# MrOlm/inStrain

Hardware: AMD Instinct MI355X
Metric: Gbp profiled/s (higher is better)
Workload: dtype u32

## Files before the change

### instrain_amd/csrc/isx_api.hip

```cpp
#include <algorithm>
#include <atomic>
#include <cmath>
#include <chrono>
#include <cstdlib>
#include <cstring>
#include <map>
#include <mutex>
#include <string>
#include <unordered_map>
#include <thread>
#include <type_traits>
#include <vector>
#include <unistd.h>
#include <sys/prctl.h>
#include <time.h>

#include "isx_batch.h"
#include "seg_encode.h"

static thread_local std::string g_err;
void isx_set_error(const std::string &msg) { g_err = msg; }

namespace {
struct BlockCache {
// ... 169 lines not shown
    std::lock_guard<std::mutex> lk(g_hreg_mu);
    for (size_t i = 0; i < g_hreg.size(); i++)
        if (g_hreg[i].a == a) {
            g_hreg.erase(g_hreg.begin() + (long)i);
            HIP_TRY(hipHostUnregister(const_cast<void *>(ptr)));
            return ISX_OK;
        }
    isx_set_error("isx_host_unregister: not a registered range");
    return ISX_ERR_ARG;
}

namespace {
__global__ void __launch_bounds__(256) k_copy_out(uint4 *__restrict__ dst, const uint4 *__restrict__ src, size_t n16)
{
    typedef uint32_t u32x4 __attribute__((ext_vector_type(4)));
    const size_t stride = (size_t)gridDim.x * blockDim.x;
    for (size_t i = (size_t)blockIdx.x * blockDim.x + threadIdx.x; i < n16; i += stride) {
        const u32x4 v = __builtin_nontemporal_load(reinterpret_cast<const u32x4 *>(src) + i);
        reinterpret_cast<u32x4 *>(dst)[i] = v;
    }
}
}

namespace {
template <class T>
__global__ void __launch_bounds__(256) k_copy_small(T *__restrict__ dst, const T *__restrict__ src, size_t n)
{
    const size_t stride = (size_t)gridDim.x * blockDim.x;
    for (size_t i = (size_t)blockIdx.x * blockDim.x + threadIdx.x; i < n; i += stride) dst[i] = src[i];
}
}

hipError_t isx_copy_to_host(void *hdst, const void *dsrc, size_t bytes, hipStream_t stream)
{
    static const size_t dma_min = [] { const char *e = getenv("ISX_D2H_DMA_MIN"); return e ? (size_t)atoll(e) : (size_t)1 << 20; }();
    return isx_copy_to_host_route(hdst, dsrc, bytes, stream, bytes < dma_min);
}

hipError_t isx_copy_to_host_route(void *hdst, const void *dsrc, size_t bytes, hipStream_t stream, bool by_kernel)
{
    if (!bytes) return hipSuccess;
    if (!by_kernel) return hipMemcpyAsync(hdst, dsrc, bytes, hipMemcpyDeviceToHost, stream);
    const uintptr_t both = reinterpret_cast<uintptr_t>(hdst) | reinterpret_cast<uintptr_t>(dsrc);
    size_t done = 0;
    if ((both & 15) == 0 && bytes >= 4096) {
        const size_t n16 = bytes / 16;
        const int blocks = (int)std::min<size_t>(128, (n16 + 1023) / 1024);
        hipLaunchKernelGGL(k_copy_out, dim3(blocks), dim3(256), 0, stream, static_cast<uint4 *>(hdst), static_cast<const uint4 *>(dsrc), n16);
        done = n16 * 16;
    }
    if (done < bytes) {
        const size_t rest = bytes - done;
        uint8_t *d = static_cast<uint8_t *>(hdst) + done;
        const uint8_t *s = static_cast<const uint8_t *>(dsrc) + done;
        const bool words = (((both | rest) & 3) == 0);
        const size_t n = words ? rest / 4 : rest;
        const int blocks = (int)std::min<size_t>(64, (n + 255) / 256);
        if (words) hipLaunchKernelGGL(k_copy_small<uint32_t>, dim3(blocks), dim3(256), 0, stream, reinterpret_cast<uint32_t *>(d), reinterpret_cast<const uint32_t *>(s), n);
        else hipLaunchKernelGGL(k_copy_small<uint8_t>, dim3(blocks), dim3(256), 0, stream, d, s, n);
    }
    return hipGetLastError();
}

namespace {
__global__ void __launch_bounds__(256) k_copy_counted(uint4 *__restrict__ dst, const uint4 *__restrict__ src, const uint32_t *cursor,
                                                      uint32_t base, uint32_t row_bytes, uint64_t cap_rows)
{
    const uint64_t rows = min((uint64_t)(*cursor - base), cap_rows);
    const uint64_t n16 = (rows * row_bytes + 15) / 16;
    const uint64_t stride = (uint64_t)gridDim.x * blockDim.x;
    for (uint64_t i = (uint64_t)blockIdx.x * blockDim.x + threadIdx.x; i < n16; i += stride) dst[i] = src[i];
}
}

hipError_t isx_copy_rows_to_host(void *hdst, const void *dsrc, const uint32_t *d_cursor, uint32_t base, uint32_t row_bytes,
                                 size_t cap_rows, hipStream_t stream)
{
    if (!cap_rows) return hipSuccess;
    if (((reinterpret_cast<uintptr_t>(hdst) | reinterpret_cast<uintptr_t>(dsrc)) & 15) != 0) return hipErrorInvalidValue;
    const size_t n16 = (cap_rows * row_bytes + 15) / 16;
    const int blocks = (int)std::min<size_t>(64, (n16 + 1023) / 1024);
    hipLaunchKernelGGL(k_copy_counted, dim3(std::max(blocks, 1)), dim3(256), 0, stream, static_cast<uint4 *>(hdst), static_cast<const uint4 *>(dsrc),
                       d_cursor, base, row_bytes, (uint64_t)cap_rows);
    return hipGetLastError();
}

namespace {
struct CopyJobs { uint4 *dst[ISX_COPY_JOBS]; const uint4 *src[ISX_COPY_JOBS]; uint32_t n16[ISX_COPY_JOBS]; uint32_t first[ISX_COPY_JOBS + 1]; int n; };
__global__ void __launch_bounds__(256) k_copy_multi(const CopyJobs J)
{
    int j = 0;
    while (j + 1 < J.n && blockIdx.x >= J.first[j + 1]) j++;
    const uint32_t nb = J.first[j + 1] - J.first[j], lb = blockIdx.x - J.first[j];
    for (uint32_t i = lb * 256u + threadIdx.x; i < J.n16[j]; i += nb * 256u) J.dst[j][i] = J.src[j][i];
}
}

hipError_t isx_copy_multi_to_host(const isx_copy_job *jobs, int n, hipStream_t stream)
{
    CopyJobs J{};
    uint32_t blocks = 0;
    for (int i = 0; i < n && J.n < ISX_COPY_JOBS; i++) {
        if (!jobs[i].bytes) continue;
        if (((reinterpret_cast<uintptr_t>(jobs[i].dst) | reinterpret_cast<uintptr_t>(jobs[i].src)) & 15) != 0 || jobs[i].bytes > ((size_t)1 << 35)) return hipErrorInvalidValue;
        const uint32_t n16 = (uint32_t)((jobs[i].bytes + 15) / 16);
        J.dst[J.n] = static_cast<uint4 *>(jobs[i].dst); J.src[J.n] = static_cast<const uint4 *>(jobs[i].src); J.n16[J.n] = n16;
        J.first[J.n] = blocks;
        blocks += std::max<uint32_t>(1, std::min<uint32_t>(64, (n16 + 1023) / 1024));
        J.n++;
    }
    if (!J.n) return hipSuccess;
    J.first[J.n] = blocks;
    hipLaunchKernelGGL(k_copy_multi, dim3(blocks), dim3(256), 0, stream, J);
    return hipGetLastError();
}

namespace {
struct ReadBack {
    uint8_t *pin = nullptr;
    size_t used = 0;
    struct Item { void *dst; size_t off, bytes; };
    std::vector<Item> items;
    bool batching = false;
    std::vector<isx_copy_job> jobs;
    static constexpr size_t CAP = (size_t)1 << 20;
    ~ReadBack() { if (pin) isx_pin_free(pin); }
};
thread_local ReadBack g_rb;
}

void isx_read_batch(bool on) { g_rb.batching = on; }

hipError_t isx_read_back(void *host_dst, const void *dsrc, size_t bytes, hipStream_t stream)
{
    if (!bytes) return hipSuccess;
    ReadBack &rb = g_rb;
    if (!rb.pin && isx_pin_malloc(reinterpret_cast<void **>(&rb.pin), ReadBack::CAP) != hipSuccess) rb.pin = nullptr;
    const size_t off = (rb.used + 15) & ~(size_t)15;
    if (!rb.pin || off + ((bytes + 15) & ~(size_t)15) > ReadBack::CAP) {
        const hipError_t e = hipMemcpyAsync(host_dst, dsrc, bytes, hipMemcpyDeviceToHost, stream);
        if (e != hipSuccess) { rb.items.clear(); rb.jobs.clear(); rb.used = 0; }
        return e;
    }
    if (rb.batching && (reinterpret_cast<uintptr_t>(dsrc) & 15) == 0 && rb.jobs.size() < ISX_COPY_JOBS) {
        rb.jobs.push_back(isx_copy_job{rb.pin + off, dsrc, bytes});
    } else {
        const hipError_t e = isx_copy_to_host(rb.pin + off, dsrc, bytes, stream);
        if (e != hipSuccess) { rb.items.clear(); rb.jobs.clear(); rb.used = 0; return e; }
    }
    rb.items.push_back({host_dst, off, bytes});
    rb.used = off + bytes;
    return hipSuccess;
}

void isx_read_drop()
{
    g_rb.items.clear();
    g_rb.jobs.clear();
    g_rb.batching = false;
    g_rb.used = 0;
}

static bool isx_active_wait()
{
    static const bool a = getenv("ISX_ACTIVE_WAIT") != nullptr;
    return a;
// ... 971 lines not shown
            HIP_TRY(isx_dev_malloc(reinterpret_cast<void **>(&b->d_win_site_base), want * sizeof(uint32_t)));
            HIP_TRY(isx_dev_malloc(reinterpret_cast<void **>(&b->d_win_site_cnt), want * sizeof(uint32_t)));
            b->cap_win_sites = want;
        }
        a.win_site_base = b->d_win_site_base; a.win_site_cnt = b->d_win_site_cnt;
    }
    launch_pileup(a, b->block, b->lds, b->grid, b->packed, s, b->ev[0], b->ev[1]);
    if (b->M == 1) {
        launch_win_order(b->d_win_rec, b->d_win_out, b->n_win, b->W, b->d_snv_raw, b->d_snv, b->d_sites_raw, b->d_sites,
                         a.clon_list, b->d_clon_sorted, b->d_rare ? b->d_rare_raw : nullptr, b->d_rare, b->d_win_out + b->cap_win * 4, b->epoch + 1, s);
        b->ordered = true;
    }
    HIP_TRY(hipGetLastError());
    ++b->epoch;
    b->publish_enqueued = false;
    c->unpublished[b->ps] = b;
    b->in_flight = true;
    return ISX_OK;
}

int finish_pass(isx_batch *b, uint32_t *cap_flags, hipStream_t link_stream)
{
    const int rc = finish_pass_sizes(b, cap_flags, link_stream);
    if (rc != ISX_OK || *cap_flags) return rc;
    return finish_pass_link(b, link_stream);
}

int finish_pass_sizes(isx_batch *b, uint32_t *cap_flags, hipStream_t link_stream)
{
    *cap_flags = 0;
    isx_ctx *c = b->ctx;
    HIP_TRY(hipSetDevice(c->device));
    hipStream_t s = link_stream ? link_stream : c->stream;
    b->in_flight = false;
    if (!b->publish_enqueued) {
        PileupArgs pa{};
        pa.cursors = b->d_cursors; pa.host_state = b->d_host_state;
        launch_publish_state(pa, b->epoch, c->pstream[b->ps]);
        b->publish_enqueued = true;
        if (c->unpublished[b->ps] == b) c->unpublished[b->ps] = nullptr;
    }
    {
        volatile uint32_t *ep = b->h_state + CUR_N + 4;
        const auto t0 = std::chrono::steady_clock::now();
        bool seen = false;
        for (;;) {
            if (__atomic_load_n(ep, __ATOMIC_ACQUIRE) == b->epoch) { seen = true; break; }
            if (std::chrono::steady_clock::now() - t0 > std::chrono::microseconds(b->spin_us)) break;
        }
        if (!seen) HIP_TRY(isx_wait_stream(c->pstream[b->ps]));
    }
    uint32_t cur[CUR_N];
    for (int i = 0; i < CUR_N; i++) { cur[i] = b->h_state[i] - b->base[i]; b->base[i] = b->h_state[i]; }
    const uint32_t flags = b->h_state[CUR_N];
    if (flags) {
        HIP_TRY(hipMemsetAsync(b->d_cursors, 0, (CUR_N + 4) * sizeof(uint32_t), s));
        HIP_TRY(isx_wait_stream(s));
        memset(b->base, 0, sizeof(b->base));
    }
    b->sites_loose = (flags & ISX_FLAG_SITES_LOOSE) != 0;
    if (flags & ISX_FLAG_MM_RANGE) { isx_set_error("an observation has mm >= n_mm_bins"); return ISX_ERR_MM_RANGE; }
    if (flags & (ISX_FLAG_CAP_ENTRIES | ISX_FLAG_CAP_SNV | ISX_FLAG_CAP_SITES | ISX_FLAG_CAP_AO)) {
        *cap_flags = flags & (ISX_FLAG_CAP_ENTRIES | ISX_FLAG_CAP_SNV | ISX_FLAG_CAP_SITES | ISX_FLAG_CAP_AO);
        return ISX_OK;
    }
    b->sizes = isx_sizes{};
    b->ld_host = nullptr; b->n_ld_host = 0; b->link_chain = 0;
    b->sizes.n_entries = cur[CUR_ENT_TOTAL];
    b->n_ovf = b->lev_sparse ? cur[CUR_ENT_TOTAL] : cur[CUR_ENTRIES];
    b->sizes.n_snv = cur[CUR_SNV];
    b->sizes.n_sites = cur[CUR_SITES];
    b->n_rare = cur[CUR_RARE]; b->n_sat = cur[CUR_SAT]; b->n_clon = cur[CUR_CLON]; b->n_cov_rows = cur[CUR_COVX];
    b->tim = isx_timings{};
    b->tim_pending = true;
    b->tim.pileup_blocks = b->grid;
    b->tim.pileup_threads = b->block;
    b->tim.pileup_lds_bytes = (int32_t)b->lds;
    b->tim.pileup_window = b->W;
    b->tim.record_bytes = b->d_seg ? 64 : (b->d_drec ? 32 : (b->d_rec16 ? 2 : (b->d_rec32 ? 4 : 8)));
    b->n_ao_pass = cur[CUR_AO];
    return ISX_OK;
}

int finish_pass_link(isx_batch *b, hipStream_t link_stream)
{
    isx_ctx *c = b->ctx;
    hipStream_t s = link_stream ? link_stream : c->stream;
    if (b->prm.enable_linkage) {
        LinkageIn in{};
        in.stream = s; in.ev = &b->ev[2]; in.ev_mfma = &b->ev[8];
        in.mode = b->prm.linkage_mode == 2 ? 2 : 1;
        in.philox = Philox{(uint32_t)b->prm.seed, (uint32_t)(b->prm.seed >> 32)};
        in.n_pairs = b->n_pairs; in.ao = b->d_ao; in.n_ao = b->n_ao_pass;
        in.sites = b->d_sites; in.n_sites = (uint32_t)b->sizes.n_sites; in.sites_ordered = b->ordered;
        in.slev = b->d_slev; in.snv = b->d_snv;
        if (b->M > 1 && b->d_win_site_cnt && !b->sites_loose) { in.win_site_base = b->d_win_site_base; in.win_site_cnt = b->d_win_site_cnt; in.n_win = b->n_win; }
        in.split_bounds = b->d_bounds; in.n_splits = b->n_splits; in.M = b->M; in.min_snp = b->prm.min_snp;
        LinkageOut lo;
        int rc = run_linkage(in, b->L, lo);
        if (rc != ISX_OK) return rc;
        if (lo.chain != 3) HIP_TRY(isx_wait_stream(s));
        b->ld_host = lo.ld_host; b->n_ld_host = (size_t)lo.n_ld_host; b->link_chain = lo.chain;
        b->sizes.n_allele_obs = (int64_t)lo.n_ao;
        b->sizes.n_increments = (int64_t)lo.n_increments;
        b->sizes.n_edges = (int64_t)lo.n_edges;
        b->sizes.n_ld = (int64_t)lo.n_ld;
        b->tim.sites_ms = ev_ms(b->ev[2], b->ev[3]);
        b->tim.allele_ms = ev_ms(b->ev[3], b->ev[4]);
        b->tim.group_ms = ev_ms(b->ev[4], b->ev[5]);
        b->tim.incr_ms = ev_ms(b->ev[5], b->ev[6]);
        b->tim.ld_ms = ev_ms(b->ev[6], b->ev[7]);
        b->tim.total_ms = ev_ms(b->ev[0], b->ev[7]);
        b->tim.mfma_ms = ev_ms(b->ev[8], b->ev[9]);
        b->tim.dense_tiles = (int32_t)lo.dense_tiles; b->tim.dense_macs = (int64_t)lo.dense_macs;
        b->tim.dense_bytes = (int64_t)lo.dense_bytes;
    } else {
        b->tim.total_ms = 0.f;
    }
    b->ran = true;
    return ISX_OK;
}

int batch_grow_tables(isx_batch *b, uint32_t cap_flags)
{
    const uint64_t pos_bound = (uint64_t)(b->cap_pos ? b->cap_pos : b->n_pos);
    const uint64_t obs_bound = (uint64_t)std::max<int64_t>(b->cap_obs ? b->cap_obs : b->n_obs, 1);
    const uint64_t npm = pos_bound * b->M;
    int rc = ISX_OK;
    HIP_TRY(hipSetDevice(b->ctx->device));
    if (cap_flags & ISX_FLAG_CAP_SNV) { if ((rc = regrow(&b->d_snv, &b->cap_snv, (size_t)npm))) return rc; }
    if (cap_flags & ISX_FLAG_CAP_SITES) {
        const bool slev_short = b->M > 1 && b->cap_slev < b->cap_sites * (size_t)b->M;
        if (b->cap_sites < (size_t)pos_bound || !slev_short) {
            if ((rc = regrow(&b->d_sites, &b->cap_sites, (size_t)pos_bound))) return rc;
        }
        if (b->M > 1) {
            if (b->d_slev) isx_dev_free(b->d_slev);
            b->d_slev = nullptr;
            b->cap_slev = b->cap_sites * (size_t)b->M;
            HIP_TRY(isx_raw_dev_malloc(&b->d_slev, b->cap_slev * sizeof(isx_slev)));
        }
    }
    if (cap_flags & ISX_FLAG_CAP_AO) { if ((rc = regrow(&b->d_ao, &b->cap_ao, (size_t)obs_bound))) return rc; }
    if ((cap_flags & ISX_FLAG_CAP_ENTRIES) && b->lev_sparse) {
        const size_t bound = (size_t)std::min<uint64_t>(npm, 0xFFFFFFF0ull);
        if (b->cap_lev >= bound) { isx_set_error("output table is at its hard bound and still too small"); return ISX_ERR_CAPACITY; }
        const size_t cap = std::min(bound, std::max<size_t>(b->cap_lev * 4, 1024));
        if (b->d_lev_cov) isx_dev_free(b->d_lev_cov);
        b->d_lev_cov = nullptr;
        HIP_TRY(isx_raw_dev_malloc(reinterpret_cast<uint8_t **>(&b->d_lev_cov), cap * 2 + 64));
        if (b->d_entries) {
            isx_dev_free(b->d_entries);
            b->d_entries = nullptr;
            HIP_TRY(isx_raw_dev_malloc(&b->d_entries, cap * sizeof(isx_entry)));
            b->cap_entries = cap;
        }
        b->cap_lev = cap;
    } else if (cap_flags & ISX_FLAG_CAP_ENTRIES) {
        const size_t used_slabs = (size_t)b->n_win * b->slab;
        const size_t slabs = b->slab_region ? b->slab_region : used_slabs;
        size_t cap = b->cap_entries - slabs;
        isx_entry *dummy = nullptr;
        if ((rc = regrow(&dummy, &cap, (size_t)npm))) return rc;
        isx_dev_free(dummy);
        if (slabs + cap >= 0xFFFFFFFFull) { isx_set_error("mm path: more than 2^32 entry slots in one batch"); return ISX_ERR_CAPACITY; }
        if (b->d_entries) isx_dev_free(b->d_entries);
        b->d_entries = nullptr;
        HIP_TRY(isx_raw_dev_malloc(&b->d_entries, (slabs + cap) * sizeof(isx_entry)));
        b->cap_entries = slabs + cap;
        b->cap_ovf = b->cap_entries - used_slabs;
    }
    return ISX_OK;
}

int isx_batch_launch(isx_batch *b)
{
    if (!b) { isx_set_error("isx_batch_launch: NULL batch"); return ISX_ERR_ARG; }
    if (b->in_flight) { isx_set_error("isx_batch_launch: the batch already has a pass in flight (isx_batch_wait first)"); return ISX_ERR_STATE; }
    return launch_pass(b);
}
// ... 372 lines not shown
```

### instrain_amd/csrc/isx_batch.h

```cpp
#pragma once
#include <vector>

#include "isx_internal.h"
#include "isx_linkage.h"
#include "isx_summary.h"

namespace isxenc { class HostPool; }

struct isx_ctx {
    int device = 0;
    hipStream_t stream = nullptr;
    hipStream_t pstream[2] = {nullptr, nullptr};
    uint32_t side_mask[8] = {0, 0, 0, 0, 0, 0, 0, 0};
    int pass_cus = 256;
    struct isx_batch *unpublished[2] = {nullptr, nullptr};
    unsigned n_created = 0;
    unsigned n_pipes = 0;
    uint8_t *d_lut = nullptr;
    std::vector<int32_t> h_lut;
    int32_t lut_n = 0, fallback = 0;
    void *pin[2] = {nullptr, nullptr};
    hipEvent_t pin_ev[2] = {nullptr, nullptr};
    size_t pin_bytes = 0;
};
// ... 40 lines not shown
    float *d_clon_r = nullptr;
    uint16_t *d_cov16 = nullptr;
    uint2 *d_rare = nullptr;
    size_t cap_rare = 0;
    uint32_t n_rare = 0, n_sat = 0;
    uint8_t *d_cov8 = nullptr;
    uint2 *d_sat = nullptr, *d_clon_list = nullptr, *d_clon_sorted = nullptr;
    size_t cap_sat = 0, cap_clon = 0;
    uint32_t n_clon = 0;
    int spin_us = 2000;
    bool nib_pass = false;
    bool nib_out = false;
    uint32_t *d_cov_row_win = nullptr;
    size_t cap_cov_row_win = 0;
    uint32_t n_cov_rows = 0;
    bool sparse_out = false, cov8_out = false;
    bool rare_dense = true;
    bool lean = false, clon_dense = false;
    bool lev_sparse = false;
    void *d_lev_mask = nullptr, *d_lev_cov = nullptr;
    uint32_t *d_lev_win_off = nullptr;
    size_t cap_lev = 0;
    int lev_mask_bytes = 0, lev_cov_bytes = 1;
    isx_entry *d_entries = nullptr;
    uint32_t *d_win_nent = nullptr;
    uint32_t *d_win_site_base = nullptr, *d_win_site_cnt = nullptr;
    size_t cap_win_sites = 0;
    bool sites_loose = false;
    isx_slev *d_slev = nullptr;
    uint32_t slab = 0;
    size_t cap_ovf = 0, cap_slev = 0;
    isx_snv *d_snv = nullptr;
    isx_site *d_sites = nullptr;
    isx_snv *d_snv_raw = nullptr;
    isx_site *d_sites_raw = nullptr;
    uint2 *d_rare_raw = nullptr;
    uint32_t *d_win_rec = nullptr, *d_win_out = nullptr;
    size_t cap_snv_raw = 0, cap_sites_raw = 0, cap_rare_raw = 0, cap_win = 0;
    bool ordered = false;
    isx_ao *d_ao = nullptr;
    uint32_t *d_cursors = nullptr, *d_flags = nullptr;
    uint32_t *h_state = nullptr;
    uint32_t *d_host_state = nullptr;
    uint32_t base[CUR_N] = {};
    uint32_t epoch = 0;
    size_t cap_entries = 0, cap_snv = 0, cap_sites = 0, cap_ao = 0;
    LinkageBuffers L;
    const isx_ld *ld_host = nullptr;
    size_t n_ld_host = 0;
    uint32_t n_ao_pass = 0;
    int link_chain = 0;
    SummaryBuffers S;
    CompareBuffers C;
    hipEvent_t ev_sum[2] = {};
    hipEvent_t ev[10] = {};
    bool ran = false;
    uint32_t n_ovf = 0;
    isx_sizes sizes{};
    isx_timings tim{};
};


static inline uint32_t entry_wins(const isx_batch *b) { return b->lev_sparse ? 0u : (uint32_t)b->n_win; }

std::vector<uint16_t> build_thresholds(const std::vector<int32_t> &lut, int32_t fallback, double min_freq);

void batch_pick_block(isx_batch *b);
int batch_window_for(const isx_batch *b, int64_t n_pos, bool packed);

int check_split_bounds(int64_t n_pos, int32_t n_splits, const int64_t *split_bounds);

int seg_status_error(int erc, const char *capacity_text, int capacity_code);

struct ChunkDir { const uint32_t *cmin, *cmax; const uint8_t *cany; uint64_t n_chunks; uint32_t chunk; };
struct DirThreads { isxenc::HostPool &pool; std::vector<uint32_t> &pmax, &smin; };
int choose_windows(const isx_batch *b, int64_t n_pos, const ChunkDir &dir, DirThreads *mt, std::vector<uint2> &win, int *packed);

int batch_set_geometry(isx_batch *b);

extern "C" {
int launch_pass(isx_batch *b);
int finish_pass(isx_batch *b, uint32_t *cap_flags, hipStream_t link_stream = nullptr);
int finish_pass_sizes(isx_batch *b, uint32_t *cap_flags, hipStream_t link_stream = nullptr);
int finish_pass_link(isx_batch *b, hipStream_t link_stream = nullptr);
int batch_grow_tables(isx_batch *b, uint32_t cap_flags);
}
```

### instrain_amd/csrc/isx_internal.h

```cpp
#pragma once
#include <hip/hip_runtime.h>
#include <stdint.h>
#include <string>

#include "../../include/instrain_amd.h"

#define ISX_PAD32 0x0700FFFFu
#define ISX_GROUP16 512
#define ISX_GROUP 256
#define ISX_CHUNK 1024
#define ISX_DENSE_PAD 8
#define ISX_SEG_GROUP 16
#define ISX_SEG_PAD 32
#define ISX_SEG_LM 16
#define ISX_PK16_MAX_W 3264
#define ISX_PAD 2048
#define ISX_SENTINEL 0xFFFFFFFFu
#define ISX_TAIL_BYTES 65536
#define ISX_TAIL_GROUPS 256

void isx_set_error(const std::string &msg);

hipError_t isx_dev_malloc(void **p, size_t bytes);
void isx_dev_free(void *p);
hipError_t isx_pin_malloc(void **p, size_t bytes);
void isx_pin_free(void *p);
void isx_dev_trim();

hipError_t isx_copy_to_host(void *hdst_pinned, const void *dsrc, size_t bytes, hipStream_t stream);
#define ISX_COPY_JOBS 8
struct isx_copy_job { void *dst; const void *src; size_t bytes; };
hipError_t isx_copy_multi_to_host(const isx_copy_job *jobs, int n, hipStream_t stream);
hipError_t isx_copy_to_host_route(void *hdst_pinned, const void *dsrc, size_t bytes, hipStream_t stream, bool by_kernel);
hipError_t isx_copy_rows_to_host(void *hdst_pinned, const void *dsrc, const uint32_t *d_cursor, uint32_t base, uint32_t row_bytes,
                                 size_t cap_rows, hipStream_t stream);
bool isx_host_is_registered(const void *ptr, size_t bytes);
hipError_t isx_read_back(void *host_dst, const void *dsrc, size_t bytes, hipStream_t stream);
hipError_t isx_read_sync(hipStream_t stream);
void isx_read_batch(bool on);
hipError_t isx_wait_event(hipEvent_t e);
hipError_t isx_wait_stream(hipStream_t s);
void isx_read_drop();
hipError_t isx_raw_dev_malloc(void **p, size_t bytes);
template <class T> static inline hipError_t isx_raw_dev_malloc(T **p, size_t bytes) { return isx_raw_dev_malloc(reinterpret_cast<void **>(p), bytes); }

#define HIP_TRY(expr)                                                                          \
    do {                                                                                       \
        hipError_t _e = (expr);                                                                \
        if (_e != hipSuccess) {                                                                \
            isx_set_error(std::string(#expr) + ": " + hipGetErrorString(_e));                  \
            isx_read_drop();                                                                   \
            return ISX_ERR_HIP;                                                                \
        }                                                                                      \
    } while (0)

#define ISX_FLAG_MM_RANGE 1u
#define ISX_FLAG_CAP_ENTRIES 2u
#define ISX_FLAG_CAP_SNV 4u
#define ISX_FLAG_CAP_SITES 8u
#define ISX_FLAG_CAP_AO 16u
#define ISX_FLAG_CAP_INCR 32u
#define ISX_FLAG_CAP_LD 64u
#define ISX_FLAG_SITES_LOOSE 128u

enum { CUR_ENTRIES = 0 , CUR_SNV = 1, CUR_SITES = 2, CUR_AO = 3, CUR_SLEV = 4,
       CUR_ENT_TOTAL = 5, CUR_RARE = 6 ,
       CUR_SAT = 7 ,
       CUR_CLON = 8 ,
       CUR_COVX = 9 , CUR_N = 10 };

struct isx_site {
    uint32_t gpos;
    uint32_t entry_off;
    uint16_t n_levels;
    uint8_t mask;
    uint8_t pad;
};

struct isx_slev {
    uint16_t mm, pad;
    uint32_t cnt[4];
};

struct isx_ao {
    uint32_t pair;
    uint32_t site;
    uint32_t obs_idx;
    uint16_t mm;
    uint8_t base;
    uint8_t pad;
};

struct Philox {
    uint32_t k0, k1;
    __host__ __device__ static inline void mulhilo(uint32_t a, uint32_t b, uint32_t &hi, uint32_t &lo)
    {
        const uint64_t p = (uint64_t)a * b;
        hi = (uint32_t)(p >> 32); lo = (uint32_t)p;
    }
    __host__ __device__ inline void operator()(uint32_t c0, uint32_t c1, uint32_t c2, uint32_t c3, uint32_t *out) const
    {
        uint32_t a = k0, b = k1;
#pragma unroll
        for (int r = 0; r < 10; r++) {
            uint32_t h0, l0, h1, l1;
            mulhilo(0xD2511F53u, c0, h0, l0);
            mulhilo(0xCD9E8D57u, c2, h1, l1);
            const uint32_t n0 = h1 ^ c1 ^ a, n1 = l1, n2 = h0 ^ c3 ^ b, n3 = l0;
            c0 = n0; c1 = n1; c2 = n2; c3 = n3;
            a += 0x9E3779B9u; b += 0xBB67AE85u;
        }
        out[0] = c0; out[1] = c1; out[2] = c2; out[3] = c3;
    }
};

__host__ __device__ inline void rarefy4(const Philox &ph, uint32_t c0, uint32_t c1, uint32_t domain, const double *p,
                                        int n_draws, uint32_t *rc)
{
// ... 107 lines not shown
```

### instrain_amd/csrc/isx_linkage.h

```cpp
#pragma once
#include <vector>
#include "isx_internal.h"

template <class T>
struct DevBuf {
    T *p = nullptr;
    size_t cap = 0;
};

constexpr size_t LD_HEAD = 1;
constexpr size_t LD_PREFIX_ROWS = 2047;

struct DenseSplit {
    uint64_t xt_off;
    uint32_t rpad;
    uint32_t ctiles;
    uint32_t first_site, n_sites, first_row;
    uint32_t tile0;
};
struct DenseTile { uint32_t slot, I, J, pad; };

struct LinkageBuffers {
    DevBuf<uint32_t> site_keys, site_keys2, site_gpos, site_split;
    DevBuf<isx_site> sites_sorted;
    DevBuf<isx_ao> ao2;
    DevBuf<uint32_t> ao_key, ao_key2;
    DevBuf<uint32_t> incr_cnt, incr_off;
    DevBuf<uint64_t> keys, keys2, ukeys;
    DevBuf<uint32_t> ucnt, n_runs, rows_per, row_off;
    DevBuf<isx_ld> ld_block;
    DevBuf<isx_ld> ld;
    DevBuf<uint8_t> temp;
    DevBuf<uint64_t> chain_head;
    DevBuf<uint32_t> next, site_cnt, site_off, site_cur, site_nu, site_rows, site_row_off, site_list1, site_list2, win_off, win_list;
    DevBuf<uint64_t> edge_list;
    uint32_t chain_epoch = 0;
    std::vector<isx_ld> h_ld;
    DevBuf<uint64_t> key64, key64b;
    DevBuf<uint32_t> head, row_id, first_row, first_site, split_slot, tile_cnt, tile_off, vals, vals2;
    DevBuf<DenseSplit> dsplits;
    DevBuf<DenseTile> dtiles;
    DevBuf<uint8_t> xt;
    void release();
};

struct LinkageIn {
    hipStream_t stream;
    hipEvent_t *ev;
    hipEvent_t *ev_mfma;
    uint64_t n_pairs;
    isx_ao *ao;
    uint32_t n_ao;
    const isx_site *sites;
    uint32_t n_sites;
    bool sites_ordered = false;
    const uint32_t *win_site_base = nullptr, *win_site_cnt = nullptr;
    int n_win = 0;
    const isx_slev *slev;
    const isx_snv *snv;
    const int64_t *split_bounds;
    int n_splits;
    int M;
    int min_snp;
    int mode;
    Philox philox;
};

struct LinkageOut {
    uint64_t n_ao = 0, n_increments = 0, n_edges = 0, n_ld = 0;
    const isx_ld *ld_host = nullptr;
    uint64_t n_ld_host = 0;
    int chain = 0;
    uint64_t dense_tiles = 0, dense_bytes = 0, dense_macs = 0;
};

int run_linkage(const LinkageIn &in, LinkageBuffers &B, LinkageOut &out);
```

### instrain_amd/csrc/isx_linkage.hip

```cpp
#include <chrono>
#include <cstdio>
#include <cstdlib>
#include <algorithm>
#include <vector>
#include <cstring>
#include <string.h>
#include <rocprim/rocprim.hpp>

#include "isx_internal.h"
#include "isx_linkage.h"

#pragma clang fp contract(off)

namespace {

__device__ __forceinline__ uint64_t make_key(int sb, uint32_t s1, uint32_t s2, uint32_t mm, uint32_t b1, uint32_t b2)
{
    return ((uint64_t)s1 << (12 + sb)) | ((uint64_t)s2 << 12) | ((uint64_t)mm << 4) | (b1 << 2) | b2;
}

__global__ void k_site_keys(const isx_site *sites, uint32_t n, uint32_t *keys)
{
    const uint32_t i = blockIdx.x * blockDim.x + threadIdx.x;
    if (i < n) keys[i] = sites[i].gpos;
// ... 142 lines not shown
        if (EMIT) {
            const double t = (double)total;
            const double fAB = (double)AB / t, fAb = (double)Ab / t, faB = (double)aB / t, fab = (double)ab / t;
            const double fA = fAB + fAb, fa = fab + faB, fB = fAB + faB, fb = fab + fAb;
            const double linkD = fAB - fA * fB;
            double r2 = __builtin_nan("");
            if (!(fa == 0 || fA == 0 || fB == 0 || fb == 0)) {
                double den = fA * fa;
                den = den * fB;
                den = den * fb;
                r2 = linkD * linkD / den;
            }
            const double linkd = fab - fa * fb;
            double dp = __builtin_nan("");
            if (linkd < 0) {
                const double d1 = (-fA) * fB, d2 = (-fa) * fb;
                dp = linkd / (d1 > d2 ? d1 : d2);
            } else if (linkD > 0) {
                const double d1 = fA * fb, d2 = fa * fB;
                dp = linkd / (d2 < d1 ? d2 : d1);
            }
            isx_ld r;
            r.gpos_a = v.sites[s1].gpos; r.gpos_b = v.sites[s2].gpos;
            r.mm = (uint16_t)mm;
            r.allele_A = (uint8_t)A; r.allele_a = (uint8_t)a; r.allele_B = (uint8_t)B; r.allele_b = (uint8_t)b;
            r.pad = 0;
            r.total = total; r.countAB = AB; r.countAb = Ab; r.countaB = aB; r.countab = ab;
            r.pad2 = 0;
            r.r2 = r2; r.d_prime = dp;
            r.r2_normalized = __builtin_nan(""); r.d_prime_normalized = __builtin_nan("");
            if (min_snp > 0) {
                const double p4[4] = {fAB, fAb, faB, fab};
                uint32_t rc[4];
                rarefy4(ph, r.gpos_a, r.gpos_b, 0x4C440000u  | mm, p4, min_snp, rc);
                const double n = (double)min_snp;
                const double gAB = (double)rc[0] / n, gAb = (double)rc[1] / n, gaB = (double)rc[2] / n, gab = (double)rc[3] / n;
                const double gA = gAB + gAb, ga = gab + gaB, gB = gAB + gaB, gb = gab + gAb;
                const double ln = gab - ga * gb;
                if (!(ga == 0 || gA == 0 || gB == 0 || gb == 0)) {
                    double den = gA * ga;
                    den = den * gB;
                    den = den * gb;
                    r.r2_normalized = ln * ln / den;
                }
                if (ln < 0) {
                    const double d1 = (-gA) * gB, d2 = (-ga) * gb;
                    r.d_prime_normalized = ln / (d1 > d2 ? d1 : d2);
                } else if (ln > 0) {
                    const double d1 = gA * gb, d2 = ga * gB;
                    r.d_prime_normalized = ln / (d2 < d1 ? d2 : d1);
                }
            }
            out[rows] = r;
        }
        rows++;
    }
    return rows;
}

template <bool EMIT>
__global__ void __launch_bounds__(256) k_ld_rows(const uint64_t *ukeys, const uint32_t *ucnt, uint32_t n_u,
                                                 SiteView v, int min_snp, uint32_t *rows_per, const uint32_t *row_off,
                                                 isx_ld *out, uint32_t *n_edges, Philox ph, int sb)
{
    const uint32_t u = blockIdx.x * blockDim.x + threadIdx.x;
    if (u >= n_u) return;
    const uint64_t k0 = ukeys[u];
    const uint64_t edge = k0 >> 12;
    const bool head = (u == 0) || ((ukeys[u - 1] >> 12) != edge);
    if (!head) { if (!EMIT) rows_per[u] = 0; return; }
    if (!EMIT) atomicAdd(n_edges, 1u);
    const uint32_t s1 = (uint32_t)(k0 >> (12 + sb)), s2 = (uint32_t)((k0 >> 12) & ((1u << sb) - 1u));
    const uint32_t rows = ld_edge_rows<EMIT>(ukeys, ucnt, u, n_u, s1, s2, v, min_snp, EMIT ? out + row_off[u] : nullptr, ph);
    if (!EMIT) rows_per[u] = rows;
}


constexpr uint32_t LK_NIL = 0xFFFFFFFFu;
constexpr int LK_SLOTS = 1024;
constexpr int LK_MAXU = 768;
constexpr uint64_t LK_EMPTY = ~0ull;
constexpr uint32_t LK_STAGE = 256;
constexpr uint32_t LK_ROUND = 16;
enum { LS_NINC = 0, LS_NU = 1, LS_NEDGES = 2, LS_NLD = 3, LS_FLAGS = 4, LS_NLIST1 = 5 , LS_NLIST2 = 6 , LS_WORDS = 16 };
constexpr uint32_t LKF_KEYS = 1u, LKF_BUCKET = 2u, LKF_LD = 4u;

__global__ void __launch_bounds__(256) k_link_prep(const isx_site *sites, uint32_t n, const int64_t *bounds, int n_splits,
                                                   uint32_t *site_gpos, uint32_t *site_split, uint32_t *site_cnt, uint32_t *site_rows, uint32_t *state)
{
    const uint32_t i = blockIdx.x * blockDim.x + threadIdx.x;
    if (i < LS_WORDS) state[i] = 0;
    if (i >= n) return;
    const uint32_t g = sites[i].gpos;
    int lo = 0, hi = n_splits;
    while (hi - lo > 1) {
        const int mid = (lo + hi) >> 1;
        if (bounds[mid] <= (int64_t)g) lo = mid; else hi = mid;
    }
    site_gpos[i] = g;
    site_split[i] = (uint32_t)lo;
    site_cnt[i] = 0;
    site_rows[i] = 0;
}

__global__ void __launch_bounds__(256) k_ao_chain(isx_ao *ao, uint32_t n, const uint32_t *site_gpos, uint32_t n_sites,
                                                  unsigned long long *head, int hshift, uint32_t direct, uint32_t epoch, uint32_t *next)
{
    const uint32_t i = blockIdx.x * blockDim.x + threadIdx.x;
    if (i >= n) return;
    const uint32_t g = ao[i].site;
    uint32_t lo = 0, hi = n_sites;
    while (lo < hi) {
        const uint32_t mid = (lo + hi) >> 1;
        if (site_gpos[mid] < g) lo = mid + 1; else hi = mid;
    }
    ao[i].site = lo;
    const uint32_t pr = ao[i].pair;
    const uint32_t h = pr < direct ? pr : (pr * 0x9E3779B1u) >> hshift;
    const unsigned long long old = atomicExch(&head[h], ((unsigned long long)epoch << 32) | i);
    next[i] = (uint32_t)(old >> 32) == epoch ? (uint32_t)old : LK_NIL;
}

template <bool EMIT>
__global__ void __launch_bounds__(256) k_pair_walk(const isx_ao *ao, uint32_t n, const uint32_t *next, const uint32_t *site_split,
                                                   uint32_t *site_cnt, const uint32_t *site_off, uint64_t *keys, uint64_t cap_keys,
                                                   uint32_t *state)
{
    const uint32_t i = blockIdx.x * blockDim.x + threadIdx.x, l = threadIdx.x & 63;
    if (EMIT && (uint64_t)state[LS_NINC] > cap_keys) {
        if (i == 0) atomicOr(&state[LS_FLAGS], LKF_KEYS);
        return;
    }
    isx_ao a{};
    uint32_t sa = 0, j = LK_NIL;
    if (i < n) { a = ao[i]; sa = site_split[a.site]; j = next[i]; }
    while (__ballot(j != LK_NIL)) {
        bool hit = false;
        uint32_t s1 = 0;
        uint64_t key = 0;
        if (j != LK_NIL) {
            const isx_ao b = ao[j];
            const uint32_t nj = next[j];
            if (b.pair == a.pair && site_split[b.site] == sa) {
                hit = true;
                const bool a_first = (a.site < b.site) || (a.site == b.site && a.obs_idx < b.obs_idx);
                s1 = a_first ? a.site : b.site;
                if (EMIT) key = a_first ? make_key(0, 0, b.site, a.mm, a.base, b.base) : make_key(0, 0, a.site, a.mm, b.base, a.base);
            }
            j = nj;
        }
        unsigned long long m = __ballot(hit);
        uint32_t slot = 0;
        while (m) {
            const int leader = __builtin_ctzll(m);
            const uint32_t ls1 = __shfl(s1, leader);
            const bool mine = hit && s1 == ls1;
            const unsigned long long same = __ballot(mine);
            uint32_t base = 0;
            if ((int)l == leader) base = atomicAdd(&site_cnt[ls1], (uint32_t)__popcll(same));
            if (EMIT) {
                base = __shfl(base, leader);
                if (mine) slot = base + (uint32_t)__popcll(same & ((1ull << l) - 1ull));
            }
            m &= ~same;
        }
        if (EMIT && hit) keys[site_off[s1] + slot] = key;
    }
}

__global__ void __launch_bounds__(1024) k_scan_u32(const uint32_t *in, uint32_t *out, uint32_t n, uint32_t *total, uint32_t *zero,
                                                   uint32_t *list, uint32_t *n_list)
{
    __shared__ uint32_t wsum[16], wnz[16];
    __shared__ uint32_t carry_s, carry_nz;
    __shared__ unsigned long long total_s;
    const uint32_t t = threadIdx.x, l = t & 63, w = t >> 6;
    if (t == 0) { carry_s = 0; carry_nz = 0; total_s = 0; }
    __syncthreads();
    auto load4 = [&](uint32_t i0) -> uint4 {
        if (i0 + 4 <= n) return *reinterpret_cast<const uint4 *>(in + i0);
        uint4 x;
        x.x = i0 < n ? in[i0] : 0u; x.y = i0 + 1 < n ? in[i0 + 1] : 0u; x.z = i0 + 2 < n ? in[i0 + 2] : 0u; x.w = 0u;
        return x;
    };
    uint4 nxt = load4(4 * t);
    for (uint32_t base = 0; base < n; base += 4096) {
        const uint32_t i0 = base + 4 * t;
        const uint4 x = nxt;
        if (base + 4096 < n) nxt = load4(i0 + 4096);
        const uint32_t v[4] = {x.x, x.y, x.z, x.w};
        const uint32_t mine = v[0] + v[1] + v[2] + v[3];
        const uint32_t mine_nz = (v[0] != 0) + (v[1] != 0) + (v[2] != 0) + (v[3] != 0);
        uint32_t inc = mine, inz = mine_nz;
#pragma unroll
        for (int d = 1; d < 64; d <<= 1) {
            const uint32_t o = __shfl_up(inc, d), oz = __shfl_up(inz, d);
            if ((int)l >= d) { inc += o; inz += oz; }
        }
        if (l == 63) { wsum[w] = inc; wnz[w] = inz; }
        __syncthreads();
        uint32_t before = carry_s, before_nz = carry_nz;
        for (uint32_t q = 0; q < w; q++) { before += wsum[q]; before_nz += wnz[q]; }
        uint32_t run = before + inc - mine, rnz = before_nz + inz - mine_nz;
        uint4 o;
        o.x = run; o.y = run + v[0]; o.z = o.y + v[1]; o.w = o.z + v[2];
        run = o.w + v[3];
        if (i0 + 4 <= n) {
            *reinterpret_cast<uint4 *>(out + i0) = o;
            if (zero) *reinterpret_cast<uint4 *>(zero + i0) = make_uint4(0, 0, 0, 0);
        } else {
            if (i0 < n) { out[i0] = o.x; if (zero) zero[i0] = 0; }
            if (i0 + 1 < n) { out[i0 + 1] = o.y; if (zero) zero[i0 + 1] = 0; }
            if (i0 + 2 < n) { out[i0 + 2] = o.z; if (zero) zero[i0 + 2] = 0; }
        }
#pragma unroll
        for (int q = 0; q < 4; q++) if (v[q] != 0) list[rnz++] = i0 + q;
        __syncthreads();
        if (t == 1023) { total_s += (unsigned long long)(run - carry_s); carry_s = run; carry_nz = rnz; }
        __syncthreads();
    }
    if (t == 0) { const uint32_t tot = total_s > 0xFFFFFFFEull ? 0xFFFFFFFFu : (uint32_t)total_s; out[n] = tot; *total = tot; *n_list = carry_nz; }
}

__device__ __forceinline__ uint32_t lk_hash(uint64_t k) { return (uint32_t)((k * 0x9E3779B97F4A7C15ull) >> 40); }

template <int G>
__device__ __forceinline__ uint64_t lk_sort_in_groups(uint64_t k, uint32_t l)
{
#pragma unroll
    for (int kk = 2; kk <= G; kk <<= 1) {
#pragma unroll
        for (int j = kk >> 1; j > 0; j >>= 1) {
            const uint64_t o = ((uint64_t)(uint32_t)__shfl_xor((int)(uint32_t)(k >> 32), j) << 32) | (uint32_t)__shfl_xor((int)(uint32_t)k, j);
            const bool up = ((l & (uint32_t)(G - 1)) & (uint32_t)kk) == 0, lower = (l & (uint32_t)j) == 0;
            k = (lower == up) ? (k < o ? k : o) : (k > o ? k : o);
        }
    }
    return k;
}

__device__ __forceinline__ void lk_flush(uint2 *stage, uint32_t &n_stage, uint2 *edge_list, uint32_t *state, uint32_t l)
{
    uint32_t eb = 0;
    if (l == 0) eb = atomicAdd(&state[LS_NEDGES], n_stage);
    eb = __shfl(eb, 0);
    __syncthreads();
    for (uint32_t q = l; q < n_stage; q += 64) edge_list[eb + q] = stage[q];
    __syncthreads();
    n_stage = 0;
}

template <int G>
__device__ __forceinline__ void lk_small_buckets(unsigned long long todo, uint32_t my_s1, uint32_t my_off, uint32_t my_nb, uint32_t l,
                                                 uint64_t *keys, uint32_t *ucnt, uint32_t *rows_per, uint32_t *site_nu, uint2 *stage,
                                                 uint32_t &n_stage, uint32_t &nu_sum, uint2 *edge_list, uint32_t *state)
{
    constexpr int NG = 64 / G;
    const uint32_t g = l / G, t = l % G;
    while (todo) {
        int src = -1;
#pragma unroll
        for (int q = 0; q < NG; q++) {
            const int sq = todo ? __builtin_ctzll(todo) : -1;
            if (todo) todo &= todo - 1;
            if ((int)g == q) src = sq;
        }
        const bool has = src >= 0;
        const int sl = has ? src : 0;
        const uint32_t s1 = __shfl(my_s1, sl), off = __shfl(my_off, sl), n_b = has ? __shfl(my_nb, sl) : 0u;
        uint64_t k = t < n_b ? keys[off + t] : LK_EMPTY;
        k = lk_sort_in_groups<G>(k, l);
        const bool valid = k != LK_EMPTY;
        const uint64_t prev = ((uint64_t)(uint32_t)__shfl_up((int)(uint32_t)(k >> 32), 1) << 32) | (uint32_t)__shfl_up((int)(uint32_t)k, 1);
        const bool uhead = valid && (t == 0 || k != prev);
        const bool ehead = uhead && (t == 0 || (k >> 12) != (prev >> 12));
        const unsigned long long ub = __ballot(uhead), eb = __ballot(ehead);
        const unsigned long long gb = G == 64 ? ub : (ub >> (g * G)) & ((1ull << (G & 63)) - 1ull);
        const uint32_t rank = (uint32_t)__popcll(gb & ((1ull << t) - 1ull));
        if (uhead) {
            const unsigned long long above = t == G - 1 ? 0ull : gb >> (t + 1);
            const uint32_t next = above ? t + 1 + (uint32_t)__builtin_ctzll(above) : n_b;
            keys[off + rank] = k;
            ucnt[off + rank] = next - t;
            rows_per[off + rank] = 0;
        }
        if (has && t == 0) site_nu[s1] = (uint32_t)__popcll(gb);
        if (n_stage + (uint32_t)__popcll(eb) > LK_STAGE) lk_flush(stage, n_stage, edge_list, state, l);
        if (ehead) stage[n_stage + (uint32_t)__popcll(eb & ((1ull << l) - 1ull))] = make_uint2(s1, rank);
        n_stage += (uint32_t)__popcll(eb);
        nu_sum += (uint32_t)__popcll(ub);
    }
}

__global__ void __launch_bounds__(64) k_site_edges(uint64_t *keys, uint32_t *ucnt, uint32_t *rows_per, const uint32_t *site_off,
                                                   uint32_t *site_nu, uint2 *edge_list, uint32_t *state, uint32_t max_u, const uint32_t *site_list)
{
    __shared__ unsigned long long tk[LK_SLOTS];
    __shared__ uint32_t tc[LK_SLOTS];
    __shared__ uint2 stage[LK_STAGE];
    __shared__ unsigned long long cmp[64];
    const uint32_t l = threadIdx.x;
    if (state[LS_FLAGS] & LKF_KEYS) return;
    const uint32_t n_list = state[LS_NLIST1];
    uint32_t n_stage = 0, nu_sum = 0;
// ... 46 lines not shown
            return;
        }
        __syncthreads();
        if (nu <= 64 && n_b < (1u << 26)) {
            uint32_t cb = 0;
            for (uint32_t r = 0; r < slots; r += 64) {
                const unsigned long long k = tk[r + l];
                const bool valid = k != LK_EMPTY;
                const unsigned long long bal = __ballot(valid);
                if (valid) cmp[cb + (uint32_t)__popcll(bal & ((1ull << l) - 1ull))] = (k << 26) | tc[r + l];
                cb += (uint32_t)__popcll(bal);
            }
            __syncthreads();
            uint64_t v = l < nu ? cmp[l] : LK_EMPTY;
            v = lk_sort_in_groups<64>(v, l);
            const bool valid = l < nu;
            const uint64_t k = v >> 26;
            const uint64_t pk = ((uint64_t)(uint32_t)__shfl_up((int)(uint32_t)(k >> 32), 1) << 32) | (uint32_t)__shfl_up((int)(uint32_t)k, 1);
            const bool head = valid && (l == 0 || (pk >> 12) != (k >> 12));
            if (valid) { keys[off + l] = k; ucnt[off + l] = (uint32_t)(v & ((1u << 26) - 1u)); rows_per[off + l] = 0; }
            const unsigned long long hb = __ballot(head);
            if (n_stage + (uint32_t)__popcll(hb) > LK_STAGE) lk_flush(stage, n_stage, edge_list, state, l);
            if (head) stage[n_stage + (uint32_t)__popcll(hb & ((1ull << l) - 1ull))] = make_uint2(s1, l);
            n_stage += (uint32_t)__popcll(hb);
            if (l == 0) site_nu[s1] = nu;
            nu_sum += nu;
            continue;
        }
        uint32_t base = 0;
        for (uint32_t r = 0; r < slots; r += 64) {
            const unsigned long long k = tk[r + l];
            const uint32_t c = tc[r + l];
            const bool valid = k != LK_EMPTY;
            const unsigned long long bal = __ballot(valid);
            const uint32_t rank = (uint32_t)__popcll(bal & ((1ull << l) - 1ull));
            __syncthreads();
            if (valid) { tk[base + rank] = k; tc[base + rank] = c; }
            base += (uint32_t)__popcll(bal);
            __syncthreads();
        }
        uint32_t n_pad = 2;
        while (n_pad < nu) n_pad <<= 1;
        for (uint32_t q = nu + l; q < n_pad; q += 64) { tk[q] = LK_EMPTY; tc[q] = 0; }
        __syncthreads();
        for (uint32_t kk = 2; kk <= n_pad; kk <<= 1) {
            for (uint32_t j = kk >> 1; j > 0; j >>= 1) {
                for (uint32_t t = l; t < n_pad / 2; t += 64) {
                    const uint32_t i = ((t & ~(j - 1)) << 1) | (t & (j - 1)), p = i | j;
                    const bool up = (i & kk) == 0;
                    const unsigned long long x = tk[i], y = tk[p];
                    if ((x > y) == up) {
                        const uint32_t cx = tc[i], cy = tc[p];
                        tk[i] = y; tk[p] = x; tc[i] = cy; tc[p] = cx;
                    }
                }
                __syncthreads();
            }
        }
        for (uint32_t c = 0; c < nu; c += 64) {
            const uint32_t u = c + l;
            bool head = false;
            if (u < nu) {
                const uint64_t k = tk[u];
                keys[off + u] = k;
                ucnt[off + u] = tc[u];
                rows_per[off + u] = 0;
                head = u == 0 || (tk[u - 1] >> 12) != (k >> 12);
            }
            const unsigned long long hb = __ballot(head);
            if (n_stage + (uint32_t)__popcll(hb) > LK_STAGE) lk_flush(stage, n_stage, edge_list, state, l);
            if (head) stage[n_stage + (uint32_t)__popcll(hb & ((1ull << l) - 1ull))] = make_uint2(s1, u);
            n_stage += (uint32_t)__popcll(hb);
        }
        if (l == 0) site_nu[s1] = nu;
        nu_sum += nu;
    }
    }
    if (n_stage) lk_flush(stage, n_stage, edge_list, state, l);
    if (l == 0 && nu_sum) atomicAdd(&state[LS_NU], nu_sum);
}

template <bool EMIT>
__global__ void __launch_bounds__(256) k_edge_rows(const uint64_t *keys, const uint32_t *ucnt, uint32_t *rows_per, const uint32_t *site_off,
                                                   const uint32_t *site_nu, uint32_t *site_rows, const uint32_t *site_row_off, const uint2 *edge_list,
                                                   SiteView v, int min_snp, isx_ld *out, uint64_t cap_ld, uint32_t *state, Philox ph)
{
    if (state[LS_FLAGS] & (LKF_KEYS | LKF_BUCKET)) return;
    if (EMIT && (uint64_t)state[LS_NLD] > cap_ld) { if (blockIdx.x == 0 && threadIdx.x == 0) atomicOr(&state[LS_FLAGS], LKF_LD); return; }
    const uint32_t n_edges = state[LS_NEDGES];
    for (uint32_t e = blockIdx.x * blockDim.x + threadIdx.x; e < n_edges; e += gridDim.x * blockDim.x) {
        const uint2 ed = edge_list[e];
        const uint32_t s1 = ed.x, u = ed.y, off = site_off[s1], nu = site_nu[s1];
        const uint32_t s2 = (uint32_t)(keys[off + u] >> 12);
        if (!EMIT) {
            const uint32_t rows = ld_edge_rows<false>(keys + off, ucnt + off, u, nu, s1, s2, v, min_snp, nullptr, ph);
            if (rows) { rows_per[off + u] = rows; atomicAdd(&site_rows[s1], rows); }
        } else {
            if (rows_per[off + u] == 0) continue;
            uint32_t before = site_row_off[s1];
            for (uint32_t q = 0; q < u; q++) before += rows_per[off + q];
            (void)ld_edge_rows<true>(keys + off, ucnt + off, u, nu, s1, s2, v, min_snp, out + before, ph);
        }
    }
}

__global__ void __launch_bounds__(64) k_site_order(const isx_site *sites, const uint32_t *win_base, const uint32_t *win_off, const uint32_t *win_list,
                                                   const uint32_t *n_list_p, isx_site *sorted)
{
    const uint32_t l = threadIdx.x, n_list = *n_list_p;
    for (uint32_t li = blockIdx.x; li < n_list; li += gridDim.x) {
        const uint32_t w = win_list[li], off = win_off[w], n = win_off[w + 1] - off;
        const isx_site *src = sites + win_base[w];
        for (uint32_t e = l; e < n; e += 64) {
            const isx_site me = src[e];
            uint32_t rank = 0;
            for (uint32_t j = 0; j < n; j++) rank += src[j].gpos < me.gpos ? 1u : 0u;
            sorted[off + rank] = me;
        }
    }
}

__global__ void k_ao_pair_keys(const isx_ao *ao, uint32_t n, uint32_t *ao_key)
{
    const uint32_t i = blockIdx.x * blockDim.x + threadIdx.x;
    if (i < n) ao_key[i] = ao[i].pair;
}


typedef int v4i __attribute__((ext_vector_type(4)));
typedef int v16i __attribute__((ext_vector_type(16)));

__global__ void k_ao_key64(const isx_ao *ao, uint32_t n, const uint32_t *site_split, uint64_t *key)
{
    const uint32_t i = blockIdx.x * blockDim.x + threadIdx.x;
    if (i < n) key[i] = ((uint64_t)site_split[ao[i].site] << 32) | ao[i].pair;
}

__global__ void k_row_heads(const uint64_t *key, uint32_t n, uint32_t *head)
{
    const uint32_t i = blockIdx.x * blockDim.x + threadIdx.x;
    if (i < n) head[i] = (i == 0 || key[i] != key[i - 1]) ? 1u : 0u;
}

__global__ void k_split_first_row(const uint64_t *key, const uint32_t *row_id, uint32_t n, uint32_t *first_row)
{
    const uint32_t i = blockIdx.x * blockDim.x + threadIdx.x;
    if (i >= n) return;
    const uint32_t sp = (uint32_t)(key[i] >> 32);
    if (i == 0 || (uint32_t)(key[i - 1] >> 32) != sp) first_row[sp] = row_id[i];
}

__global__ void k_split_first_site(const uint32_t *site_split, uint32_t n_sites, uint32_t *first_site)
{
    const uint32_t i = blockIdx.x * blockDim.x + threadIdx.x;
    if (i >= n_sites) return;
    if (i == 0 || site_split[i - 1] != site_split[i]) first_site[site_split[i]] = i;
}

__global__ void k_dense_scatter(const isx_ao *ao, const uint64_t *key, const uint32_t *row_id, const uint32_t *head,
                                uint32_t n, const uint32_t *split_slot, const DenseSplit *splits, uint8_t *xt)
{
    const uint32_t i = blockIdx.x * blockDim.x + threadIdx.x;
    if (i >= n) return;
    const uint32_t slot = split_slot[(uint32_t)(key[i] >> 32)];
    if (slot == 0xFFFFFFFFu) return;
    const DenseSplit ds = splits[slot];
    const isx_ao a = ao[i];
    const uint64_t row = row_id[i] + head[i] - 1 - ds.first_row;
    const uint64_t col = (uint64_t)(a.site - ds.first_site) * 4 + a.base;
    const uint64_t idx = ds.xt_off + col * ds.rpad + row;
    atomicAdd(reinterpret_cast<uint32_t *>(xt + (idx & ~3ull)), 1u << (8 * (idx & 3)));
}

constexpr int DG_LDS_BYTES = 2 * 2 * 128 * 128;

template <bool EMIT>
__global__ void __launch_bounds__(256) k_dense_gemm(const DenseTile *blocks, const DenseSplit *splits, const uint8_t *xt,
                                                    uint32_t *tile_cnt, const uint32_t *tile_off, uint64_t *keys,
                                                    uint32_t *cnts, int sb)
{
    extern __shared__ __attribute__((aligned(16))) uint8_t dg_lds[];
    const DenseTile bl = blocks[blockIdx.x];
    const DenseSplit ds = splits[bl.slot];
    const int tid = threadIdx.x, l = tid & 63, wave = __builtin_amdgcn_readfirstlane(tid >> 6), wi = wave >> 1, wj = wave & 1;
    const uint32_t ncols = ds.ctiles * 32;
// ... 119 lines not shown
    const int rc = ensure(B.ld_block, n + LD_HEAD);
    if (rc) return rc;
    B.ld.p = B.ld_block.p + LD_HEAD;
    B.ld.cap = B.ld_block.cap - LD_HEAD;
    return ISX_OK;
}

inline int bits_for(uint64_t n)
{
    int b = 1;
    while (b < 64 && (n >> b)) b++;
    return b;
}

}

void LinkageBuffers::release()
{
    void *ps[] = {site_keys.p, site_keys2.p, sites_sorted.p, site_gpos.p, site_split.p, ao_key.p, ao2.p,
                  ao_key2.p, incr_cnt.p, incr_off.p, keys.p, keys2.p, ukeys.p, ucnt.p, n_runs.p, rows_per.p,
                  row_off.p, ld_block.p, temp.p, chain_head.p, next.p, site_cnt.p, site_off.p, site_cur.p, site_nu.p, site_rows.p, site_row_off.p, site_list1.p, site_list2.p, edge_list.p, win_off.p, win_list.p, key64.p, key64b.p, head.p, row_id.p, first_row.p, first_site.p,
                  split_slot.p, tile_cnt.p, tile_off.p, vals.p, vals2.p, dsplits.p, dtiles.p, xt.p};
    for (void *p : ps) if (p) isx_dev_free(p);
    *this = LinkageBuffers();
}

using isx_sort_onesweep = rocprim::radix_sort_config<rocprim::default_config, rocprim::default_config, rocprim::default_config, 0>;
static const bool g_sort_merge = getenv("ISX_SORT_MERGE") != nullptr;
#define EV(i) HIP_TRY(hipEventRecord(in.ev[i], s))
#define RP(call_with_temp)                                                                       \
    do {                                                                                         \
        void *tp = nullptr; size_t tb = 0;                                                       \
        HIP_TRY(call_with_temp);                                                                 \
        if ((rc = ensure_temp(B.temp, tb))) return rc;                                           \
        tp = B.temp.p; tb = B.temp.cap;                                                          \
        HIP_TRY(call_with_temp);                                                                 \
    } while (0)

namespace {

int scan_total(LinkageBuffers &B, hipStream_t s, uint32_t *cnt, uint32_t *off, uint32_t n, uint64_t &total)
{
    int rc;
    RP(rocprim::exclusive_scan(tp, tb, cnt, off, 0u, n, rocprim::plus<uint32_t>(), s));
    uint32_t last_off = 0, last_cnt = 0;
    HIP_TRY(isx_read_back(&last_off, off + (n - 1), 4, s));
    HIP_TRY(isx_read_back(&last_cnt, cnt + (n - 1), 4, s));
    HIP_TRY(isx_read_sync(s));
    total = (uint64_t)last_off + last_cnt;
    return ISX_OK;
}

int sparse_path(const LinkageIn &in, LinkageBuffers &B, LinkageOut &out, uint32_t n_ao, uint32_t &n_u)
{
    hipStream_t s = in.stream;
    int rc;
    const int sb = bits_for(in.n_sites);
    n_u = 0;
    const int pair_bits = bits_for(in.n_pairs ? in.n_pairs : 0xFFFFFFFFull);
    if (g_sort_merge) RP(rocprim::radix_sort_pairs(tp, tb, B.ao_key.p, B.ao_key2.p, in.ao, B.ao2.p, n_ao, 0, pair_bits, s));
    else RP(rocprim::radix_sort_pairs<isx_sort_onesweep>(tp, tb, B.ao_key.p, B.ao_key2.p, in.ao, B.ao2.p, n_ao, 0, pair_bits, s));
    EV(3);
    if ((rc = ensure(B.incr_cnt, n_ao)) || (rc = ensure(B.incr_off, (size_t)n_ao + 1))) return rc;
    hipLaunchKernelGGL((k_pair_incr<false, false>), dim3((n_ao + 255) / 256), dim3(256), 0, s, B.ao2.p, n_ao,
                       B.site_split.p, B.incr_cnt.p, nullptr, nullptr, sb);
    uint64_t n_inc = 0;
    if ((rc = scan_total(B, s, B.incr_cnt.p, B.incr_off.p, n_ao, n_inc))) return rc;
    out.n_increments = n_inc;
    if (n_inc == 0) { EV(4); return ISX_OK; }
    if (n_inc >= 0xFFFFFFFFull) { isx_set_error("more than 2^32 pair increments in one batch"); return ISX_ERR_CAPACITY; }
    if ((rc = ensure(B.keys, n_inc)) || (rc = ensure(B.keys2, n_inc)) || (rc = ensure(B.ukeys, n_inc)) ||
        (rc = ensure(B.ucnt, n_inc)) || (rc = ensure(B.n_runs, 2))) return rc;
    hipLaunchKernelGGL((k_pair_incr<true, false>), dim3((n_ao + 255) / 256), dim3(256), 0, s, B.ao2.p, n_ao,
                       B.site_split.p, nullptr, B.incr_off.p, B.keys.p, sb);
    if (g_sort_merge) RP(rocprim::radix_sort_keys(tp, tb, B.keys.p, B.keys2.p, (size_t)n_inc, 0, 2 * sb + 12, s));
    else RP(rocprim::radix_sort_keys<isx_sort_onesweep>(tp, tb, B.keys.p, B.keys2.p, (size_t)n_inc, 0, 2 * sb + 12, s));
    RP(rocprim::run_length_encode(tp, tb, B.keys2.p, (size_t)n_inc, B.ukeys.p, B.ucnt.p, B.n_runs.p, s));
    HIP_TRY(isx_read_back(&n_u, B.n_runs.p, 4, s));
    EV(4);
    HIP_TRY(isx_read_sync(s));
    return ISX_OK;
}

int bucket_chain(const LinkageIn &in, LinkageBuffers &B, LinkageOut &out, const isx_site *sites_sorted, bool *fell_back)
{
    hipStream_t s = in.stream;
    int rc;
    *fell_back = false;
    const uint32_t n_ao = in.n_ao, n_sites = in.n_sites;
    const bool direct = in.n_pairs && in.n_pairs <= 8ull * n_ao + (1ull << 20) && in.n_pairs <= (1ull << 31);
    int logH = 12;
    while (logH < 31 && (1ull << logH) < (direct ? in.n_pairs : 2ull * n_ao)) logH++;
    const size_t H = (size_t)1 << logH;
    if (B.chain_head.cap < H || !B.chain_head.p) {
        if ((rc = ensure(B.chain_head, H))) return rc;
        HIP_TRY(hipMemsetAsync(B.chain_head.p, 0, B.chain_head.cap * sizeof(uint64_t), s));
        B.chain_epoch = 0;
    }
    if (++B.chain_epoch == 0) {
        HIP_TRY(hipMemsetAsync(B.chain_head.p, 0, B.chain_head.cap * sizeof(uint64_t), s));
        B.chain_epoch = 1;
    }
    size_t cap_keys = std::max<size_t>(B.keys.cap, std::max<size_t>((size_t)n_ao * 2, 65536));
    size_t cap_ld = std::max<size_t>(B.ld_block.cap > LD_HEAD ? B.ld_block.cap - LD_HEAD : 0, 4096);
    static_assert(sizeof(isx_ld) * LD_HEAD >= LS_WORDS * sizeof(uint32_t), "the state words fit the head of ld_block");
    uint32_t max_u = LK_MAXU;
    if (const char *e = getenv("ISX_LINK_MAXU")) max_u = (uint32_t)std::min<long>(std::max<long>(atol(e), 1), LK_MAXU);
    size_t test_keys = 0, test_ld = 0;
    if (const char *e = getenv("ISX_LINK_TEST_CAPS")) { unsigned long a = 0, b = 0; if (sscanf(e, "%lu,%lu", &a, &b) == 2) { test_keys = a; test_ld = b; } }
    auto size_tables = [&]() -> int {
        int r;
        if ((r = ensure(B.keys, cap_keys)) || (r = ensure(B.ucnt, cap_keys)) || (r = ensure(B.rows_per, cap_keys)) || (r = ensure(B.edge_list, cap_keys))) return r;
        cap_keys = std::min(std::min(B.keys.cap, B.ucnt.cap), std::min(B.rows_per.cap, B.edge_list.cap));
        return ISX_OK;
    };
    auto size_ld = [&]() -> int {
        const int r = ensure_ld(B, cap_ld);
        if (r) return r;
        cap_ld = B.ld.cap;
        return ISX_OK;
    };
    if ((rc = ensure(B.next, n_ao)) || (rc = ensure(B.site_cnt, (size_t)n_sites + 1)) || (rc = ensure(B.site_off, (size_t)n_sites + 1)) ||
        (rc = ensure(B.site_cur, (size_t)n_sites + 1)) || (rc = ensure(B.site_nu, n_sites)) || (rc = ensure(B.site_rows, (size_t)n_sites + 1)) ||
        (rc = ensure(B.site_row_off, (size_t)n_sites + 1)) || (rc = ensure(B.site_list1, n_sites)) || (rc = ensure(B.site_list2, n_sites)) || (rc = size_tables()) || (rc = size_ld())) return rc;
    uint32_t *state = reinterpret_cast<uint32_t *>(B.ld_block.p);
    const dim3 blk(256), g_sites((n_sites + 255) / 256), g_ao((n_ao + 255) / 256);
    SiteView v{sites_sorted, in.slev, in.snv, in.M == 1 ? 1 : 0};
    hipLaunchKernelGGL(k_link_prep, g_sites, blk, 0, s, sites_sorted, n_sites, in.split_bounds, in.n_splits, B.site_gpos.p, B.site_split.p,
                       B.site_cnt.p, B.site_rows.p, state);
    EV(1);
    hipLaunchKernelGGL(k_ao_chain, g_ao, blk, 0, s, in.ao, n_ao, B.site_gpos.p, n_sites, reinterpret_cast<unsigned long long *>(B.chain_head.p),
                       32 - logH, direct ? (uint32_t)H : 0u, B.chain_epoch, B.next.p);
    EV(2);
    hipLaunchKernelGGL((k_pair_walk<false>), g_ao, blk, 0, s, in.ao, n_ao, B.next.p, B.site_split.p, B.site_cnt.p, nullptr, nullptr, (uint64_t)0, state);
    hipLaunchKernelGGL(k_scan_u32, dim3(1), dim3(1024), 0, s, B.site_cnt.p, B.site_off.p, n_sites, state + LS_NINC, B.site_cur.p, B.site_list1.p, state + LS_NLIST1);
    const dim3 g_waves(std::min<uint32_t>((n_sites + LK_ROUND - 1) / LK_ROUND, 4096)), g_edges(std::min<uint32_t>((uint32_t)std::min<size_t>((cap_keys + 255) / 256, 0x7FFFFFFF), 2048));
    uint32_t h[LS_WORDS] = {0};
    for (int stage = 0, attempt = 0;; attempt++) {
        if (attempt == 4) { isx_set_error("linkage tables still too small after three growth steps"); return ISX_ERR_CAPACITY; }
        if (stage == 0) {
            hipLaunchKernelGGL((k_pair_walk<true>), g_ao, blk, 0, s, in.ao, n_ao, B.next.p, B.site_split.p, B.site_cur.p, B.site_off.p, B.keys.p,
                               (uint64_t)(attempt == 0 && test_keys ? std::min(test_keys, cap_keys) : cap_keys), state);
            EV(3);
            hipLaunchKernelGGL(k_site_edges, g_waves, dim3(64), 0, s, B.keys.p, B.ucnt.p, B.rows_per.p, B.site_off.p, B.site_nu.p,
                               reinterpret_cast<uint2 *>(B.edge_list.p), state, max_u, B.site_list1.p);
            hipLaunchKernelGGL((k_edge_rows<false>), g_edges, blk, 0, s, B.keys.p, B.ucnt.p, B.rows_per.p, B.site_off.p, B.site_nu.p, B.site_rows.p,
                               (const uint32_t *)nullptr, reinterpret_cast<const uint2 *>(B.edge_list.p), v, in.min_snp, (isx_ld *)nullptr, (uint64_t)0, state, in.philox);
            hipLaunchKernelGGL(k_scan_u32, dim3(1), dim3(1024), 0, s, B.site_rows.p, B.site_row_off.p, n_sites, state + LS_NLD, (uint32_t *)nullptr, B.site_list2.p, state + LS_NLIST2);
            EV(4);
        }
        hipLaunchKernelGGL((k_edge_rows<true>), g_edges, blk, 0, s, B.keys.p, B.ucnt.p, B.rows_per.p, B.site_off.p, B.site_nu.p, B.site_rows.p,
                           B.site_row_off.p, reinterpret_cast<const uint2 *>(B.edge_list.p), v, in.min_snp, B.ld.p,
                           (uint64_t)(attempt == 0 && test_ld ? std::min(test_ld, cap_ld) : cap_ld), state, in.philox);
        HIP_TRY(hipGetLastError());
        const size_t n_pre = std::min<size_t>(cap_ld, LD_PREFIX_ROWS);
        B.h_ld.resize(LD_HEAD + n_pre);
        HIP_TRY(isx_read_back(B.h_ld.data(), B.ld_block.p, (LD_HEAD + n_pre) * sizeof(isx_ld), s));
        EV(5);
        HIP_TRY(isx_read_sync(s));
        memcpy(h, B.h_ld.data(), sizeof(h));
        if (h[LS_FLAGS] & LKF_KEYS) {
            if (h[LS_NINC] == 0xFFFFFFFFu) { isx_set_error("more than 2^32 pair increments in one batch"); return ISX_ERR_CAPACITY; }
            cap_keys = (size_t)h[LS_NINC] + h[LS_NINC] / 4 + 4096;
            B.keys.cap = B.ucnt.cap = B.rows_per.cap = B.edge_list.cap = 0;
            if ((rc = size_tables())) return rc;
            HIP_TRY(hipMemsetAsync(state + LS_NU, 0, (LS_FLAGS + 1 - LS_NU) * sizeof(uint32_t), s));
            HIP_TRY(hipMemsetAsync(B.site_cur.p, 0, ((size_t)n_sites + 1) * sizeof(uint32_t), s));
            stage = 0;
            continue;
        }
        if (h[LS_FLAGS] & LKF_BUCKET) { *fell_back = true; return ISX_OK; }
        if (h[LS_FLAGS] & LKF_LD) {
            if (h[LS_NLD] == 0xFFFFFFFFu) { isx_set_error("more than 2^32 LD rows in one batch"); return ISX_ERR_CAPACITY; }
            cap_ld = (size_t)h[LS_NLD] + h[LS_NLD] / 4 + 4096;
            B.ld_block.cap = 0;
            if ((rc = size_ld())) return rc;
            state = reinterpret_cast<uint32_t *>(B.ld_block.p);
            h[LS_FLAGS] &= ~LKF_LD;
            HIP_TRY(hipMemcpyAsync(state, h, sizeof(h), hipMemcpyHostToDevice, s));
            HIP_TRY(isx_wait_stream(s));
            stage = 1;
            continue;
        }
        break;
    }
    out.n_increments = h[LS_NINC];
    out.n_edges = h[LS_NEDGES];
    out.n_ld = h[LS_NLD];
    out.ld_host = B.h_ld.data() + LD_HEAD;
    out.n_ld_host = std::min<uint64_t>(out.n_ld, B.h_ld.size() - LD_HEAD);
    return ISX_OK;
}

int dense_path(const LinkageIn &in, LinkageBuffers &B, LinkageOut &out, uint32_t n_ao, uint32_t n_sites, uint32_t &n_u)
{
    hipStream_t s = in.stream;
    int rc;
    n_u = 0;
    const int sb = bits_for(n_sites);
    const uint32_t nsp = (uint32_t)in.n_splits;
    if ((rc = ensure(B.key64, n_ao)) || (rc = ensure(B.key64b, n_ao)) || (rc = ensure(B.head, n_ao)) ||
        (rc = ensure(B.row_id, (size_t)n_ao + 1)) || (rc = ensure(B.first_row, (size_t)nsp + 1)) ||
        (rc = ensure(B.first_site, (size_t)nsp + 1)) || (rc = ensure(B.split_slot, nsp))) return rc;
    const dim3 ga((n_ao + 255) / 256), blk(256);
    hipLaunchKernelGGL(k_ao_key64, ga, blk, 0, s, in.ao, n_ao, B.site_split.p, B.key64.p);
    const int key_bits = 32 + bits_for(nsp);
    RP(rocprim::radix_sort_pairs(tp, tb, B.key64.p, B.key64b.p, in.ao, B.ao2.p, n_ao, 0, key_bits, s));
    EV(3);
    hipLaunchKernelGGL(k_row_heads, ga, blk, 0, s, B.key64b.p, n_ao, B.head.p);
    uint64_t n_rows = 0;
    if ((rc = scan_total(B, s, B.head.p, B.row_id.p, n_ao, n_rows))) return rc;
    HIP_TRY(hipMemsetAsync(B.first_row.p, 0xFF, ((size_t)nsp + 1) * 4, s));
    HIP_TRY(hipMemsetAsync(B.first_site.p, 0xFF, ((size_t)nsp + 1) * 4, s));
    hipLaunchKernelGGL(k_split_first_row, ga, blk, 0, s, B.key64b.p, B.row_id.p, n_ao, B.first_row.p);
    hipLaunchKernelGGL(k_split_first_site, dim3((n_sites + 255) / 256), blk, 0, s, B.site_split.p, n_sites, B.first_site.p);
    std::vector<uint32_t> frow((size_t)nsp + 1), fsite((size_t)nsp + 1);
    HIP_TRY(isx_read_back(frow.data(), B.first_row.p, frow.size() * 4, s));
    HIP_TRY(isx_read_back(fsite.data(), B.first_site.p, fsite.size() * 4, s));
    HIP_TRY(isx_read_sync(s));
    frow[nsp] = (uint32_t)n_rows; fsite[nsp] = n_sites;
    for (uint32_t i = nsp; i-- > 0;) {
        if (frow[i] == 0xFFFFFFFFu) frow[i] = frow[i + 1];
        if (fsite[i] == 0xFFFFFFFFu) fsite[i] = fsite[i + 1];
    }
    std::vector<DenseSplit> ds;
    std::vector<DenseTile> blocks;
    std::vector<uint32_t> slot(nsp, 0xFFFFFFFFu);
    uint64_t bytes = 0, macs = 0, n_tiles64 = 0;
    for (uint32_t sp = 0; sp < nsp; sp++) {
        const uint32_t rows = frow[sp + 1] - frow[sp], ns = fsite[sp + 1] - fsite[sp];
        if (rows == 0 || ns < 2) continue;
        DenseSplit d{};
        d.xt_off = bytes;
        d.rpad = (rows + 127) / 128 * 128;
        d.ctiles = (ns * 4 + 31) / 32;
        d.first_site = fsite[sp]; d.n_sites = ns; d.first_row = frow[sp];
        d.tile0 = (uint32_t)n_tiles64;
        bytes += (uint64_t)d.ctiles * 32 * d.rpad;
        slot[sp] = (uint32_t)ds.size();
        const uint32_t nb = (d.ctiles + 3) / 4;
        for (uint32_t I = 0; I < nb; I++)
            for (uint32_t J = I; J < nb; J++) blocks.push_back(DenseTile{(uint32_t)ds.size(), I, J, 0});
        n_tiles64 += (uint64_t)d.ctiles * (d.ctiles + 1) / 2;
        macs += (uint64_t)d.ctiles * (d.ctiles + 1) / 2 * 32 * 32 * d.rpad;
        ds.push_back(d);
    }
    out.dense_tiles = n_tiles64; out.dense_bytes = bytes; out.dense_macs = macs;
    if (bytes > (16ull << 30)) { isx_set_error("dense linkage path needs > 16 GiB for X^T: use the sparse path"); return ISX_ERR_CAPACITY; }
    if (n_tiles64 >= 0xFFFFFFFFull || blocks.size() >= 0x7FFFFFFFull) { isx_set_error("too many dense tiles"); return ISX_ERR_CAPACITY; }
    const uint32_t n_tiles = (uint32_t)n_tiles64, n_blocks = (uint32_t)blocks.size();
    uint64_t n_gemm = 0;
    if (n_tiles) {
        if ((rc = ensure(B.dsplits, ds.size())) || (rc = ensure(B.dtiles, blocks.size())) || (rc = ensure(B.xt, bytes + 16)) ||
            (rc = ensure(B.tile_cnt, n_tiles)) || (rc = ensure(B.tile_off, (size_t)n_tiles + 1))) return rc;
        HIP_TRY(hipMemcpyAsync(B.dsplits.p, ds.data(), ds.size() * sizeof(DenseSplit), hipMemcpyHostToDevice, s));
        HIP_TRY(hipMemcpyAsync(B.dtiles.p, blocks.data(), blocks.size() * sizeof(DenseTile), hipMemcpyHostToDevice, s));
        HIP_TRY(hipMemcpyAsync(B.split_slot.p, slot.data(), slot.size() * 4, hipMemcpyHostToDevice, s));
        HIP_TRY(hipMemsetAsync(B.xt.p, 0, bytes + 16, s));
        hipLaunchKernelGGL(k_dense_scatter, ga, blk, 0, s, B.ao2.p, B.key64b.p, B.row_id.p, B.head.p, n_ao, B.split_slot.p,
                           B.dsplits.p, B.xt.p);
        HIP_TRY(hipEventRecord(in.ev_mfma[0], s));
        (void)hipFuncSetAttribute(reinterpret_cast<const void *>(&k_dense_gemm<false>), hipFuncAttributeMaxDynamicSharedMemorySize, DG_LDS_BYTES);
        (void)hipFuncSetAttribute(reinterpret_cast<const void *>(&k_dense_gemm<true>), hipFuncAttributeMaxDynamicSharedMemorySize, DG_LDS_BYTES);
        hipLaunchKernelGGL((k_dense_gemm<false>), dim3(n_blocks), blk, DG_LDS_BYTES, s, B.dtiles.p, B.dsplits.p,
                           B.xt.p, B.tile_cnt.p, nullptr, nullptr, nullptr, sb);
        HIP_TRY(hipEventRecord(in.ev_mfma[1], s));
        if ((rc = scan_total(B, s, B.tile_cnt.p, B.tile_off.p, n_tiles, n_gemm))) return rc;
    } else {
        HIP_TRY(hipEventRecord(in.ev_mfma[0], s));
        HIP_TRY(hipEventRecord(in.ev_mfma[1], s));
    }
    if ((rc = ensure(B.incr_cnt, n_ao)) || (rc = ensure(B.incr_off, (size_t)n_ao + 1))) return rc;
    hipLaunchKernelGGL((k_pair_incr<false, true>), ga, blk, 0, s, B.ao2.p, n_ao, B.site_split.p, B.incr_cnt.p, nullptr, nullptr, sb);
    uint64_t n_self = 0;
    if ((rc = scan_total(B, s, B.incr_cnt.p, B.incr_off.p, n_ao, n_self))) return rc;
    const uint64_t n_k = n_gemm + n_self;
    if (n_k == 0) { EV(4); return ISX_OK; }
    if (n_k >= 0xFFFFFFFFull) { isx_set_error("more than 2^32 co-occurrence keys in one batch"); return ISX_ERR_CAPACITY; }
    if ((rc = ensure(B.keys, n_k)) || (rc = ensure(B.keys2, n_k)) || (rc = ensure(B.vals, n_k)) || (rc = ensure(B.vals2, n_k)) ||
        (rc = ensure(B.ukeys, n_k)) || (rc = ensure(B.ucnt, n_k)) || (rc = ensure(B.n_runs, 2))) return rc;
    if (n_gemm)
        hipLaunchKernelGGL((k_dense_gemm<true>), dim3(n_blocks), blk, DG_LDS_BYTES, s, B.dtiles.p, B.dsplits.p, B.xt.p,
                           nullptr, B.tile_off.p, B.keys.p, B.vals.p, sb);
    if (n_self) {
        hipLaunchKernelGGL((k_pair_incr<true, true>), ga, blk, 0, s, B.ao2.p, n_ao, B.site_split.p, nullptr, B.incr_off.p,
                           B.keys.p + n_gemm, sb);
        hipLaunchKernelGGL(k_fill_ones, dim3(((uint32_t)n_self + 255) / 256), blk, 0, s, B.vals.p + n_gemm, (uint32_t)n_self);
    }
    RP(rocprim::radix_sort_pairs(tp, tb, B.keys.p, B.keys2.p, B.vals.p, B.vals2.p, (size_t)n_k, 0, 2 * sb + 12, s));
    RP(rocprim::reduce_by_key(tp, tb, B.keys2.p, B.vals2.p, (size_t)n_k, B.ukeys.p, B.ucnt.p, B.n_runs.p,
                              rocprim::plus<uint32_t>(), rocprim::equal_to<uint64_t>(), s));
    RP(rocprim::reduce(tp, tb, B.vals2.p, B.n_runs.p + 1, 0u, (size_t)n_k, rocprim::plus<uint32_t>(), s));
    uint32_t h2[2] = {0, 0};
    HIP_TRY(isx_read_back(h2, B.n_runs.p, 8, s));
    EV(4);
    HIP_TRY(isx_read_sync(s));
    n_u = h2[0];
    out.n_increments = h2[1];
    return ISX_OK;
}

}

int run_linkage(const LinkageIn &in, LinkageBuffers &B, LinkageOut &out)
{
    hipStream_t s = in.stream;
    out = LinkageOut();
    const uint32_t n_sites = in.n_sites;
    int rc;
    const bool lt = getenv("ISX_LINK_TIMING") != nullptr;
    const auto lt0 = std::chrono::steady_clock::now();
    auto tick = [&](const char *what) {
        if (lt) fprintf(stderr, "[run_linkage] %-22s +%.2f ms\n", what, std::chrono::duration<double, std::milli>(std::chrono::steady_clock::now() - lt0).count());
    };
    EV(0);
    HIP_TRY(hipEventRecord(in.ev_mfma[0], s));
    HIP_TRY(hipEventRecord(in.ev_mfma[1], s));
    if (n_sites == 0) { EV(1); EV(2); EV(3); EV(4); EV(5); return ISX_OK; }
    if (n_sites >= (1u << 26)) { isx_set_error("more than 2^26 SNP sites in one batch: split the batch"); return ISX_ERR_ARG; }
    if (in.M > 256) { isx_set_error("linkage supports at most 256 mm bins"); return ISX_ERR_ARG; }
    if (in.mode == 2 && in.M != 1) { isx_set_error("the dense MFMA linkage path needs n_mm_bins == 1"); return ISX_ERR_ARG; }

    if ((rc = ensure(B.site_keys, n_sites)) || (rc = ensure(B.site_keys2, n_sites)) ||
        (rc = ensure(B.sites_sorted, n_sites)) || (rc = ensure(B.site_gpos, n_sites)) ||
        (rc = ensure(B.site_split, n_sites))) return rc;
    tick("site buffers");
    const isx_site *sites_sorted = in.sites;
    const char *site_env = getenv("ISX_LINK_SITE_SORT");
    if (!in.sites_ordered && in.win_site_cnt && in.n_win > 0 && !(site_env && !strcmp(site_env, "rocprim"))) {
        if ((rc = ensure(B.win_off, (size_t)in.n_win + 1)) || (rc = ensure(B.win_list, (size_t)in.n_win)) || (rc = ensure(B.n_runs, 2))) return rc;
        hipLaunchKernelGGL(k_scan_u32, dim3(1), dim3(1024), 0, s, in.win_site_cnt, B.win_off.p, (uint32_t)in.n_win, B.n_runs.p, (uint32_t *)nullptr, B.win_list.p, B.n_runs.p + 1);
        hipLaunchKernelGGL(k_site_order, dim3(std::min<uint32_t>((uint32_t)in.n_win, 4096)), dim3(64), 0, s, in.sites, in.win_site_base, B.win_off.p, B.win_list.p,
                           B.n_runs.p + 1, B.sites_sorted.p);
        sites_sorted = B.sites_sorted.p;
    } else if (!in.sites_ordered) {
        hipLaunchKernelGGL(k_site_keys, dim3((n_sites + 255) / 256), dim3(256), 0, s, in.sites, n_sites, B.site_keys.p);
        RP(rocprim::radix_sort_pairs(tp, tb, B.site_keys.p, B.site_keys2.p, const_cast<isx_site *>(in.sites),
                                     B.sites_sorted.p, n_sites, 0, 32, s));
        sites_sorted = B.sites_sorted.p;
    }
    const uint32_t n_ao = in.n_ao;
    out.n_ao = n_ao;
    const char *chain_env = getenv("ISX_LINK_CHAIN");
    const bool bucket = in.mode != 2 && n_ao != 0 && !(chain_env && !strcmp(chain_env, "sorted"));
    bool ranked = false;
    if (bucket) {
        bool fell_back = false;
        if ((rc = bucket_chain(in, B, out, sites_sorted, &fell_back)) != ISX_OK) return rc;
        tick("bucket chain");
        if (!fell_back) { out.chain = 3; return ISX_OK; }
        ranked = true;
    } else {
        hipLaunchKernelGGL(k_site_split, dim3((n_sites + 255) / 256), dim3(256), 0, s, sites_sorted, n_sites,
                           in.split_bounds, in.n_splits, B.site_gpos.p, B.site_split.p);
        tick("site sort enqueued");
        EV(1);
    }
    if (n_ao == 0) { EV(2); EV(3); EV(4); EV(5); return ISX_OK; }
    if ((rc = ensure(B.ao_key, n_ao)) || (rc = ensure(B.ao2, n_ao)) || (rc = ensure(B.ao_key2, n_ao))) return rc;
    tick("ao buffers");
    if (ranked) hipLaunchKernelGGL(k_ao_pair_keys, dim3((n_ao + 255) / 256), dim3(256), 0, s, in.ao, n_ao, B.ao_key.p);
    else hipLaunchKernelGGL(k_ao_rank, dim3((n_ao + 255) / 256), dim3(256), 0, s, in.ao, n_ao, B.site_gpos.p, n_sites, B.ao_key.p);
    EV(2);
    out.chain = in.mode == 2 ? 2 : 1;

    uint32_t n_u = 0;
    if (in.mode == 2) rc = dense_path(in, B, out, n_ao, n_sites, n_u);
    else rc = sparse_path(in, B, out, n_ao, n_u);
    if (rc != ISX_OK) return rc;
    tick("pair counts");
    if (n_u == 0) { if (out.n_increments == 0) {  } EV(5); return ISX_OK; }

    const int sb = bits_for(n_sites);
    if ((rc = ensure(B.rows_per, n_u)) || (rc = ensure(B.row_off, (size_t)n_u + 1))) return rc;
    HIP_TRY(hipMemsetAsync(B.n_runs.p + 1, 0, 4, s));
    SiteView v{sites_sorted, in.slev, in.snv, in.M == 1 ? 1 : 0};
    hipLaunchKernelGGL(k_ld_rows<false>, dim3((n_u + 255) / 256), dim3(256), 0, s, B.ukeys.p, B.ucnt.p, n_u, v,
                       in.min_snp, B.rows_per.p, nullptr, nullptr, B.n_runs.p + 1, in.philox, sb);
    uint64_t n_ld = 0;
    if ((rc = scan_total(B, s, B.rows_per.p, B.row_off.p, n_u, n_ld))) return rc;
    uint32_t n_edges = 0;
    HIP_TRY(isx_read_back(&n_edges, B.n_runs.p + 1, 4, s));
    HIP_TRY(isx_read_sync(s));
    out.n_edges = n_edges;
    out.n_ld = n_ld;
    if (n_ld) {
        if ((rc = ensure_ld(B, n_ld))) return rc;
        hipLaunchKernelGGL(k_ld_rows<true>, dim3((n_u + 255) / 256), dim3(256), 0, s, B.ukeys.p, B.ucnt.p, n_u, v,
                           in.min_snp, nullptr, B.row_off.p, B.ld.p, nullptr, in.philox, sb);
    }
    EV(5);
    tick("ld rows enqueued");
    return ISX_OK;
}
```

### instrain_amd/csrc/isx_pipe.hip

```cpp
#include <atomic>
#include <algorithm>
#include <chrono>
#include <cmath>
#include <condition_variable>
#include <cstring>
#include <deque>
#include <mutex>
#include <memory>
#include <string>
#include <thread>
#include <vector>

#include "bam_front.h"
#include "isx_batch.h"
#include "obs_encode.h"
#include "seg_encode.h"
#include "isx_summary.h"
#include <unordered_map>

namespace {

constexpr size_t ALIGN = 256;
inline size_t up(size_t v, size_t a = ALIGN) { return (v + a - 1) / a * a; }

double now_ms()
{
    return std::chrono::duration<double, std::milli>(std::chrono::steady_clock::now().time_since_epoch()).count();
}

int host_block_alloc(void **p, size_t bytes, bool pinned)
{
    *p = nullptr;
    if (pinned) { HIP_TRY(isx_pin_malloc(p, std::max<size_t>(bytes, 1))); return ISX_OK; }
    if (posix_memalign(p, 4096, std::max<size_t>(bytes, 4096)) != 0) { *p = nullptr; isx_set_error("out of host memory"); return ISX_ERR_ARG; }
    return ISX_OK;
}

void host_block_free(void *p, bool pinned)
{
    if (!p) return;
    if (pinned) isx_pin_free(p); else free(p);
}

static const bool pipe_timing = getenv("ISX_PIPE_TIMING") != nullptr;
#define H2D(p, s) ((s).h2d ? (s).h2d : (p)->s_h2d)
struct Slot {
    isx_batch *b = nullptr;
    hipStream_t h2d = nullptr;
    uint8_t *h_in = nullptr, *d_in = nullptr;
    size_t in_bytes = 0;
    size_t off_bounds = 0, off_win = 0, off_ref = 0, off_gbase = 0, off_ridx = 0, off_rec = 0;
    size_t off_pairs = 0;
    isxenc::PairRun *h_runs = nullptr;
    bool runs_pinned = true;
    uint2 *d_runs = nullptr;
    size_t cap_runs = 0;
    hipEvent_t ev_ring[2] = {nullptr, nullptr};
    bool ring_busy[2] = {false, false};
    uint8_t *h_out = nullptr;
    uint8_t *h_small = nullptr;
    size_t small_bytes = 0;
    bool out_pinned = true;
    size_t out_bytes = 0, o_counts = 0, o_clon = 0, o_clonr = 0, o_snv = 0, o_cov16 = 0, o_rare = 0;
    bool rare_dense = false;
    bool cov8 = false, clon_sparse = false;
    bool cov4 = false;
    size_t cov_rows_off = 0;
    int cov_window = 0;
    std::vector<uint32_t> cov_row_win;
    std::vector<isx_sat> sat_rows;
    bool sat_complete = true;
    void *sort_temp = nullptr;
    size_t sort_temp_bytes = 0;
    std::vector<float> clonr_big;
    std::vector<isx_rare> rare_big;
    std::vector<uint32_t> cmin, cmax, dir_pmax, dir_smin;
    std::vector<uint8_t> cany;
    std::vector<uint2> win;
    size_t o_lmask = 0, o_lwin = 0, o_lcov = 0, o_lclon = 0, o_lrare = 0;
    size_t lcov_room = 0, lclon_room = 0, lrare_room = 0;
    std::vector<uint8_t> lcov_big;
    std::vector<isx_rare> lclon_big, lrare_big;
    std::vector<isx_snv> snv_big;
    std::vector<isx_ld> ld_rows;
    uint64_t rows_checksum = 0;
    hipEvent_t ev_h2d0 = nullptr, ev_h2d1 = nullptr, ev_pass = nullptr, ev_d2h0 = nullptr, ev_d2h1 = nullptr;
    hipEvent_t ev_h2da = nullptr, ev_h2db = nullptr;
    bool h2d_split = false;
    int64_t ticket = -1;
    BamBatch *dead_batch = nullptr;
    bool ref_has_n = false;
    int state = 0;
    int rc = 0;
    std::string err;
    float finish_wait_ms = 0.f;
    float encode_ms = 0.f;
    int encode_passes = 0;
    int64_t h2d_bytes = 0, d2h_bytes = 0;
    uint16_t *d_gpos16 = nullptr;
};

static uint64_t bytes_checksum(const void *p, size_t bytes, uint64_t seed)
{
    const uint8_t *b = static_cast<const uint8_t *>(p);
    uint64_t a[4] = {seed ^ 0x9E3779B97F4A7C15ull, seed + 0xC2B2AE3D27D4EB4Full, seed ^ 0x165667B19E3779F9ull, seed + 0x27D4EB2F165667C5ull};
    const size_t n8 = bytes / 8;
    size_t i = 0;
    for (; i + 4 <= n8; i += 4) {
        uint64_t w[4];
        memcpy(w, b + 8 * i, 32);
        for (int k = 0; k < 4; k++) a[k] = a[k] * 0x100000001B3ull + w[k];
    }
    uint64_t h = (uint64_t)bytes;
    for (; i < n8; i++) { uint64_t w; memcpy(&w, b + 8 * i, 8); h = h * 0x100000001B3ull + w; }
    for (size_t j = n8 * 8; j < bytes; j++) h = h * 0x100000001B3ull + b[j];
    for (int k = 0; k < 4; k++) { h ^= a[k]; h *= 0xFF51AFD7ED558CCDull; h ^= h >> 33; }
    return h;
}

static inline size_t ref2_bytes(int64_t n_pos) { return (((size_t)n_pos + 3) / 4 + 15) & ~(size_t)15; }
static inline size_t refn_bytes(int64_t n_pos) { return (((size_t)n_pos + 7) / 8 + 15) & ~(size_t)15; }

static bool copy_ref_planes(isxenc::HostPool &pool, const isx_ref_planes *rp, int64_t n_pos, uint8_t *plane2, uint8_t *nplane)
{
    const size_t b2 = ((size_t)n_pos + 3) / 4, bn = ((size_t)n_pos + 7) / 8;
    const size_t piece = (size_t)1 << 20;
    const int t2 = (int)((b2 + piece - 1) / piece), tn = rp->nplane ? (int)((bn + piece - 1) / piece) : 0;
    std::atomic<int> any{0};
    pool.run(t2 + tn, [&](int t) {
        if (t < t2) { const size_t a = (size_t)t * piece; memcpy(plane2 + a, rp->plane2 + a, std::min(piece, b2 - a)); return; }
        const size_t a = (size_t)(t - t2) * piece, n = std::min(piece, bn - a);
        const uint8_t *src = rp->nplane + a;
        uint8_t acc = 0;
        for (size_t i = 0; i < n; i++) acc |= src[i];
        memcpy(nplane + a, src, n);
        if (acc) any.store(1, std::memory_order_relaxed);
    });
    return any.load() != 0;
}

static bool plane_any(isxenc::HostPool &pool, const uint8_t *pl, size_t bytes)
{
    const size_t piece = (size_t)1 << 20;
    const int nt = (int)((bytes + piece - 1) / piece);
    std::atomic<int> any{0};
    pool.run(nt, [&](int t) {
// ... 236 lines not shown
        else {
            b->cap_clon = (size_t)cap_pos / 2 + 65536;
            HIP_TRY(isx_dev_malloc(reinterpret_cast<void **>(&b->d_cov8), (size_t)cap_pos));
            if (p->pp.lean_output) {
                b->cap_cov_row_win = (size_t)cap_pos / 64 + 2;
                HIP_TRY(isx_dev_malloc(reinterpret_cast<void **>(&b->d_cov_row_win), b->cap_cov_row_win * sizeof(uint32_t)));
            }
            HIP_TRY(isx_dev_malloc(reinterpret_cast<void **>(&b->d_clon_list), b->cap_clon * sizeof(uint2)));
            HIP_TRY(isx_dev_malloc(reinterpret_cast<void **>(&b->d_clon_sorted), b->cap_clon * sizeof(uint2)));
        }
        b->cap_sat = (size_t)cap_pos / 16 + 65536;
        HIP_TRY(isx_dev_malloc(reinterpret_cast<void **>(&b->d_sat), b->cap_sat * sizeof(uint2)));
        HIP_TRY(isx_dev_malloc(reinterpret_cast<void **>(&b->d_clon), (size_t)cap_pos * sizeof(float)));
        HIP_TRY(isx_dev_malloc(reinterpret_cast<void **>(&b->d_clon_r), (size_t)cap_pos * sizeof(float)));
        HIP_TRY(isx_dev_malloc(reinterpret_cast<void **>(&b->d_cov16), (size_t)cap_pos * sizeof(uint16_t)));
        if (prm->rarefied_coverage > 0) {
            b->cap_rare = p->cap_rare;
            HIP_TRY(isx_dev_malloc(reinterpret_cast<void **>(&b->d_rare), b->cap_rare * sizeof(uint2)));
        }
    } else if (b->lev_sparse) {
        b->lev_mask_bytes = b->M <= 8 ? 1 : (b->M <= 16 ? 2 : 4);
        b->cap_lev = (size_t)std::min<uint64_t>(std::min<uint64_t>(npm, 0xFFFFFFF0ull), std::max<uint64_t>((uint64_t)cap_pos * (uint64_t)std::min(b->M, 4), 1u << 20));
        HIP_TRY(isx_dev_malloc(&b->d_lev_mask, (size_t)cap_pos * b->lev_mask_bytes + 64));
        HIP_TRY(isx_dev_malloc(&b->d_lev_cov, b->cap_lev * 2 + 64));
        HIP_TRY(isx_dev_malloc(reinterpret_cast<void **>(&b->d_lev_win_off), ((size_t)cap_pos / 64 + 2) * sizeof(uint32_t)));
        if (!b->lean) {
            b->cap_entries = b->cap_lev;
            HIP_TRY(isx_dev_malloc(reinterpret_cast<void **>(&b->d_entries), b->cap_entries * sizeof(isx_entry)));
        }
        b->cap_clon = (size_t)cap_pos / 4 + 65536;
        HIP_TRY(isx_dev_malloc(reinterpret_cast<void **>(&b->d_clon_list), b->cap_clon * sizeof(uint2)));
        b->cap_sat = (size_t)cap_pos / 16 + 65536;
        HIP_TRY(isx_dev_malloc(reinterpret_cast<void **>(&b->d_sat), b->cap_sat * sizeof(uint2)));
        if (prm->rarefied_coverage > 0) {
            b->cap_rare = p->cap_rare;
            HIP_TRY(isx_dev_malloc(reinterpret_cast<void **>(&b->d_rare), b->cap_rare * sizeof(uint2)));
        }
    } else {
        b->slab_region = (size_t)(cap_pos + 2 * b->block) * (size_t)std::min(b->M, 4);
        const size_t ovf = b->M <= 4 ? 16 : (size_t)std::max<uint64_t>(1u << 20, std::min<uint64_t>(cap_obs, npm) / 4);
        if (b->slab_region + ovf >= 0xFFFFFFFFull) { isx_set_error("mm path: more than 2^32 entry slots in one batch"); return ISX_ERR_ARG; }
        b->cap_entries = b->slab_region + ovf;
        HIP_TRY(isx_dev_malloc(reinterpret_cast<void **>(&b->d_entries), b->cap_entries * sizeof(isx_entry)));
        HIP_TRY(isx_dev_malloc(reinterpret_cast<void **>(&b->d_win_nent), ((size_t)cap_pos / 64 + 2) * sizeof(uint32_t)));
    }
    b->cap_snv = (size_t)std::min<uint64_t>(npm, std::max<uint64_t>((uint64_t)cap_pos / 2, 1u << 20));
    b->cap_sites = (size_t)std::min<uint64_t>((uint64_t)cap_pos, std::max<uint64_t>((uint64_t)cap_pos / 4, 1u << 20));
    b->cap_ao = (size_t)std::max<uint64_t>(1, std::min<uint64_t>(cap_obs, std::max<uint64_t>(cap_obs / 4, 1u << 20)));
    HIP_TRY(isx_dev_malloc(reinterpret_cast<void **>(&b->d_snv), b->cap_snv * sizeof(isx_snv)));
    HIP_TRY(isx_dev_malloc(reinterpret_cast<void **>(&b->d_sites), b->cap_sites * sizeof(isx_site)));
    if (prm->enable_linkage) HIP_TRY(isx_dev_malloc(reinterpret_cast<void **>(&b->d_ao), b->cap_ao * sizeof(isx_ao)));
    if (!dense) {
        b->cap_slev = b->cap_sites * (size_t)std::min(b->M, 8);
        HIP_TRY(isx_dev_malloc(reinterpret_cast<void **>(&b->d_slev), b->cap_slev * sizeof(isx_slev)));
    }
    size_t o = 0;
    s.off_bounds = o; o = up(o + (size_t)(p->pp.max_splits + 1) * sizeof(int64_t));
    s.off_win = o; o = up(o + ((size_t)cap_pos / 64 + 2) * sizeof(uint2));
    s.off_ref = o; o = up(o + ref2_bytes(cap_pos) + refn_bytes(cap_pos));
    s.off_gbase = o; o = up(o + ((size_t)(p->cap_rec / p->G) + ISX_TAIL_GROUPS) * sizeof(uint32_t));
    s.off_ridx = o; if (prm->enable_linkage && !p->segs) o = up(o + ((size_t)p->cap_rec / ISX_CHUNK + 2) * sizeof(uint32_t));
    s.off_pairs = o; if (prm->enable_linkage && p->segs && !p->drec) o = up(o + (size_t)p->cap_rec * sizeof(uint32_t));
    s.off_rec = o;
    s.in_bytes = up(o + (size_t)p->cap_rec * p->rb + ISX_TAIL_BYTES);
    const size_t host_bytes = p->ring_half ? up(o + 2 * (size_t)p->ring_half * p->rb) : s.in_bytes;
    const double t_a0 = now_ms();
    HIP_TRY(isx_pin_malloc(reinterpret_cast<void **>(&s.h_in), host_bytes));
    const double t_a1 = now_ms();
    HIP_TRY(isx_dev_malloc(reinterpret_cast<void **>(&s.d_in), s.in_bytes));
    if (pipe_timing)
        fprintf(stderr, "[isx_pipe_create] slot %d: device tables %.1f ms, pinned input %.1f MB %.1f ms, device arena %.1f MB %.1f ms\n", index,
                t_a0 - t_s0, host_bytes / 1e6, t_a1 - t_a0, s.in_bytes / 1e6, now_ms() - t_a1);
    if (prm->enable_linkage && !p->segs) {
        s.cap_runs = (size_t)p->cap_rec / 64 + 4096;
        s.runs_pinned = p->pp.depth > 1;
        { const int hrc = host_block_alloc(reinterpret_cast<void **>(&s.h_runs), s.cap_runs * sizeof(isxenc::PairRun), s.runs_pinned); if (hrc != ISX_OK) return hrc; }
        HIP_TRY(isx_dev_malloc(reinterpret_cast<void **>(&s.d_runs), s.cap_runs * sizeof(uint2)));
    }
    if (p->ring_half) for (hipEvent_t &e : s.ev_ring) HIP_TRY(hipEventCreateWithFlags(&e, hipEventDisableTiming));
    if (prm->enable_linkage && p->rb == 4) HIP_TRY(isx_dev_malloc(reinterpret_cast<void **>(&s.d_gpos16), (size_t)p->cap_rec * sizeof(uint16_t)));
    o = 0;
    s.o_snv = o; o = up(o + p->snv_prefix * sizeof(isx_snv));
    s.o_rare = o; if (dense && prm->rarefied_coverage > 0) o = up(o + p->rare_prefix * sizeof(isx_rare));
    s.small_bytes = o;
    HIP_TRY(isx_pin_malloc(reinterpret_cast<void **>(&s.h_small), std::max<size_t>(s.small_bytes, 1)));
    o = 0;
    if (dense) {
        s.o_cov16 = o; o = up(o + (size_t)cap_pos * 2);
        s.o_clon = o; o = up(o + (size_t)cap_pos * 4);
        if (p->pp.want_counts) {
            s.o_counts = o; o = up(o + (size_t)cap_pos * 16);
            s.o_clonr = o; if (prm->rarefied_coverage > 0) o = up(o + (size_t)cap_pos * 4);
        }
    }
    if (b->lev_sparse) {
        s.o_lmask = o; o = up(o + (size_t)cap_pos * b->lev_mask_bytes);
        s.o_lwin = o; o = up(o + ((size_t)cap_pos / 64 + 2) * sizeof(uint32_t));
        s.lcov_room = (size_t)cap_pos * (size_t)std::min(b->M, 4);
        s.o_lcov = o; o = up(o + s.lcov_room);
        s.lclon_room = (size_t)cap_pos;
        s.o_lclon = o; o = up(o + s.lclon_room);
        s.lrare_room = prm->rarefied_coverage > 0 ? (size_t)cap_pos / 2 : 0;
        s.o_lrare = o; o = up(o + s.lrare_room);
    }
    s.out_bytes = o;
    const double t_o0 = now_ms();
    s.out_pinned = s.out_bytes <= ((size_t)64 << 20) || p->pp.depth > 2;
    { const int hrc = host_block_alloc(reinterpret_cast<void **>(&s.h_out), s.out_bytes, s.out_pinned); if (hrc != ISX_OK) return hrc; }
    if (pipe_timing) fprintf(stderr, "[isx_pipe_create] slot %d: %s results %.1f MB %.1f ms\n", index, s.out_pinned ? "pinned" : "pageable", s.out_bytes / 1e6, now_ms() - t_o0);
    for (hipEvent_t *e : {&s.ev_h2d0, &s.ev_h2d1, &s.ev_pass, &s.ev_d2h0, &s.ev_d2h1, &s.ev_h2da, &s.ev_h2db}) HIP_TRY(hipEventCreate(e));
    const size_t n_chunks = (size_t)(p->cap_rec / (p->segs ? (int64_t)p->G : (int64_t)ISX_CHUNK)) + 2;
    s.cmin.resize(n_chunks); s.cmax.resize(n_chunks); s.cany.resize(n_chunks);
    return ISX_OK;
}

static int finish_slot(isx_pipe *p, Slot &s, hipStream_t sfin)
{
    isx_ctx *c = p->ctx;
    isx_batch *b = s.b;
    const bool dense = b->M == 1;
    const double t0 = now_ms();
    HIP_TRY(isx_wait_event(s.ev_d2h1));
    s.finish_wait_ms = (float)(now_ms() - t0);
    const double t_c0 = now_ms();
    double t_fin = 0, t_rare = 0;
    hipStream_t ps = c->pstream[b->ps];
    bool redo = false;
    for (int attempt = 0;; attempt++) {
        uint32_t cf = 0;
        int rc = finish_pass_sizes(b, &cf, sfin);
        if (rc != ISX_OK) return rc;
        const bool cov8_overflow = !cf && dense && b->sparse_out && b->cov8_out && !b->nib_pass && (size_t)b->n_sat > b->cap_sat;
        const bool nib_overflow = !cf && dense && b->nib_pass &&
                                  ((size_t)b->n_pos / 2 + 128 + (size_t)b->n_cov_rows * (size_t)b->W * 2 > (size_t)b->n_pos * 2 ||
                                   ((size_t)b->n_cov_rows + 1) * (size_t)b->W > (size_t)(b->cap_pos ? b->cap_pos : b->n_pos));
        const bool clon_overflow = !cf && dense && b->sparse_out && b->lean && !b->clon_dense &&
                                   ((size_t)b->n_clon > b->cap_clon || (size_t)b->n_clon * 2 > (size_t)b->n_pos);
        const bool rare_overflow = !cf && dense && p->prm.rarefied_coverage > 0 && !b->rare_dense &&
                                   ((size_t)b->n_rare > p->cap_rare || (size_t)b->n_rare * 8 > (size_t)b->n_pos);
        const bool lev_overflow = !cf && b->lev_sparse && ((size_t)b->n_clon > b->cap_clon || (size_t)b->n_sat > b->cap_sat ||
                                                           (p->prm.rarefied_coverage > 0 && (size_t)b->n_rare > b->cap_rare));
        if (!cf && !cov8_overflow && !clon_overflow && !nib_overflow && !rare_overflow && !lev_overflow) break;
        if (attempt == 7) { isx_set_error("output tables still too small after 8 growth steps"); return ISX_ERR_CAPACITY; }
        if (cov8_overflow) b->cov8_out = false;
        if (nib_overflow) b->nib_out = false;
        if (clon_overflow) b->clon_dense = true;
        if (rare_overflow) b->rare_dense = true;
        if (cf && (rc = batch_grow_tables(b, cf)) != ISX_OK) return rc;
        if (lev_overflow) {
            auto regrow_list = [&](uint2 **lp, size_t *cap, size_t need) -> int {
                if (need <= *cap) return ISX_OK;
                HIP_TRY(isx_wait_stream(ps));
                if (*lp) isx_dev_free(*lp);
                *lp = nullptr;
                const size_t want = need + need / 4 + 65536;
                HIP_TRY(isx_dev_malloc(reinterpret_cast<void **>(lp), want * sizeof(uint2)));
                *cap = want;
                return ISX_OK;
            };
            if ((rc = regrow_list(&b->d_clon_list, &b->cap_clon, b->n_clon)) != ISX_OK) return rc;
            if ((rc = regrow_list(&b->d_sat, &b->cap_sat, b->n_sat)) != ISX_OK) return rc;
            if (p->prm.rarefied_coverage > 0 && (rc = regrow_list(&b->d_rare, &b->cap_rare, b->n_rare)) != ISX_OK) return rc;
        }
        if (!dense && !b->lev_sparse) b->cap_ovf = b->cap_entries - (size_t)b->n_win * b->slab;
        std::lock_guard<std::mutex> lk(p->launch_mu);
        if (dense && p->prm.rarefied_coverage > 0 && b->rare_dense)
            HIP_TRY(hipMemsetD32Async(reinterpret_cast<hipDeviceptr_t>(b->d_clon_r), 0x7FC00000, (size_t)b->n_pos, ps));
        if ((rc = launch_pass(b)) != ISX_OK) return rc;
        {
            PileupArgs pa{};
            pa.cursors = b->d_cursors; pa.host_state = b->d_host_state;
            launch_publish_state(pa, b->epoch, ps);
            b->publish_enqueued = true;
            if (c->unpublished[b->ps] == b) c->unpublished[b->ps] = nullptr;
        }
        redo = true;
    }
    s.d2h_bytes += (int64_t)(std::min((size_t)b->sizes.n_snv, p->snv_prefix) * sizeof(isx_snv));
    if (dense && p->prm.rarefied_coverage > 0) s.d2h_bytes += (int64_t)(std::min((size_t)b->n_rare, p->rare_prefix) * sizeof(isx_rare));
    auto pull = [&](void *hdst, const void *dsrc, size_t bytes) -> int {
        if (!bytes) return ISX_OK;
        HIP_TRY(isx_read_back(hdst, dsrc, bytes, sfin));
        HIP_TRY(isx_read_sync(sfin));
        return ISX_OK;
    };
    struct ReadBatch { ReadBatch() { isx_read_batch(true); } ~ReadBatch() { isx_read_drop(); } } read_batch;
    auto fetch = [&](void *hdst, const void *dsrc, size_t bytes) -> int {
        if (!bytes) return ISX_OK;
        if (!s.out_pinned) return bounce_d2h(p, hdst, dsrc, bytes, sfin);
        HIP_TRY(isx_copy_to_host(hdst, dsrc, bytes, sfin));
        return ISX_OK;
    };
    if (dense) {
        int rc = ISX_OK;
        if (redo) HIP_TRY(isx_wait_stream(ps));
        s.cov8 = false; s.cov4 = false; s.clon_sparse = false; s.sat_complete = (size_t)b->n_sat <= b->cap_sat;
        if (b->sparse_out) {
            s.cov8 = b->cov8_out && !b->nib_pass;
            if (b->nib_pass) {
                const size_t nib_bytes = ((size_t)b->n_pos + 1) / 2, rows_bytes = (size_t)b->n_cov_rows * (size_t)b->W * 2;
                s.cov4 = true; s.cov_window = b->W;
                s.cov_rows_off = (nib_bytes + 63) & ~(size_t)63;
                rc = fetch(s.h_out + s.o_cov16, b->d_cov8, nib_bytes);
                if (rc == ISX_OK) rc = fetch(s.h_out + s.o_cov16 + s.cov_rows_off, b->d_cov16, rows_bytes);
                s.cov_row_win.resize(b->n_cov_rows);
                if (rc == ISX_OK && b->n_cov_rows && isx_read_back(s.cov_row_win.data(), b->d_cov_row_win, (size_t)b->n_cov_rows * sizeof(uint32_t), sfin) != hipSuccess) {
                    isx_set_error("isx_pipe finisher: read-back of the coverage rows' windows"); isx_read_drop(); rc = ISX_ERR_HIP;
                }
                s.d2h_bytes += (int64_t)(nib_bytes + rows_bytes + (size_t)b->n_cov_rows * 4);
            } else if (s.cov8) rc = fetch(s.h_out + s.o_cov16, b->d_cov8, (size_t)b->n_pos);
            else rc = fetch(s.h_out + s.o_cov16, b->d_cov16, (size_t)b->n_pos * 2);
            if (rc != ISX_OK) return rc;
            if (!s.cov4) s.d2h_bytes += (int64_t)b->n_pos * (s.cov8 ? 1 : 2);
            const size_t n_clon = b->n_clon;
            if (n_clon <= b->cap_clon && n_clon * 2 <= (size_t)b->n_pos) {
                if (!b->ordered && (rc = sort_pairs_by_position(sfin, b->d_clon_list, b->d_clon_sorted, n_clon, &s.sort_temp, &s.sort_temp_bytes)) != ISX_OK) return rc;
                if ((rc = fetch(s.h_out + s.o_clon, b->d_clon_sorted, n_clon * sizeof(isx_rare))) != ISX_OK) return rc;
                s.clon_sparse = true;
                s.d2h_bytes += (int64_t)(n_clon * sizeof(isx_rare));
            } else {
                if ((rc = fetch(s.h_out + s.o_clon, b->d_clon, (size_t)b->n_pos * 4)) != ISX_OK) return rc;
                s.d2h_bytes += (int64_t)b->n_pos * 4;
            }
        } else if (!s.out_pinned || redo) {
            if ((rc = fetch(s.h_out + s.o_cov16, b->d_cov16, (size_t)b->n_pos * 2)) != ISX_OK) return rc;
            if ((rc = fetch(s.h_out + s.o_clon, b->d_clon, (size_t)b->n_pos * 4)) != ISX_OK) return rc;
            if (p->pp.want_counts) {
                if ((rc = fetch(s.h_out + s.o_counts, b->d_counts, (size_t)b->n_pos * 16)) != ISX_OK) return rc;
                if (p->prm.rarefied_coverage > 0 && (rc = fetch(s.h_out + s.o_clonr, b->d_clon_r, (size_t)b->n_pos * 4)) != ISX_OK) return rc;
            }
        }
        s.sat_rows.resize(s.sat_complete ? (size_t)b->n_sat : 0);
        if (!s.sat_rows.empty()) HIP_TRY(isx_read_back(s.sat_rows.data(), b->d_sat, s.sat_rows.size() * sizeof(isx_sat), sfin));
    }
    if (b->lev_sparse) {
        if (redo) HIP_TRY(isx_wait_stream(ps));
        int rc = ISX_OK;
        const size_t n_lev = (size_t)b->sizes.n_entries, cov_bytes = n_lev * (size_t)b->lev_cov_bytes;
        const size_t clon_bytes = (size_t)b->n_clon * sizeof(isx_rare), rare_bytes = p->prm.rarefied_coverage > 0 ? (size_t)b->n_rare * sizeof(isx_rare) : 0;
        static const size_t lev_kernel_max = [] { const char *e = getenv("ISX_LEV_KERNEL_MAX"); return e ? (size_t)atoll(e) : (size_t)32 << 20; }();
        const bool lev_by_kernel = s.out_pinned && (size_t)b->n_pos * b->lev_mask_bytes + cov_bytes + clon_bytes + rare_bytes <= lev_kernel_max;
        std::vector<isx_copy_job> jobs;
        auto fetch_lev = [&](void *hdst, const void *dsrc, size_t bytes) -> int {
            if (!lev_by_kernel || ((reinterpret_cast<uintptr_t>(hdst) | reinterpret_cast<uintptr_t>(dsrc)) & 15)) return fetch(hdst, dsrc, bytes);
            jobs.push_back(isx_copy_job{hdst, dsrc, bytes});
            return ISX_OK;
        };
        if ((rc = fetch_lev(s.h_out + s.o_lmask, b->d_lev_mask, (size_t)b->n_pos * b->lev_mask_bytes)) != ISX_OK) return rc;
        if ((rc = fetch_lev(s.h_out + s.o_lwin, b->d_lev_win_off, (size_t)b->n_win * sizeof(uint32_t))) != ISX_OK) return rc;
        auto fetch_or_big = [&](size_t off, size_t room, auto &big, const void *dsrc, size_t bytes) -> int {
            big.clear();
            if (bytes <= room) return fetch_lev(s.h_out + off, dsrc, bytes);
            big.resize((bytes + sizeof(big[0]) - 1) / sizeof(big[0]));
            if (p->bounce[0]) return bounce_d2h(p, big.data(), dsrc, bytes, sfin);
            HIP_TRY(hipMemcpy(big.data(), dsrc, bytes, hipMemcpyDeviceToHost));
            return ISX_OK;
        };
        if ((rc = fetch_or_big(s.o_lcov, s.lcov_room, s.lcov_big, b->d_lev_cov, cov_bytes)) != ISX_OK) return rc;
        if ((rc = fetch_or_big(s.o_lclon, s.lclon_room, s.lclon_big, b->d_clon_list, clon_bytes)) != ISX_OK) return rc;
        if (rare_bytes && (rc = fetch_or_big(s.o_lrare, s.lrare_room, s.lrare_big, b->d_rare, rare_bytes)) != ISX_OK) return rc;
        if (!jobs.empty()) HIP_TRY(isx_copy_multi_to_host(jobs.data(), (int)jobs.size(), sfin));
        s.sat_rows.resize((size_t)b->n_sat);
        if (!s.sat_rows.empty()) HIP_TRY(isx_read_back(s.sat_rows.data(), b->d_sat, s.sat_rows.size() * sizeof(isx_sat), sfin));
        s.d2h_bytes += (int64_t)((size_t)b->n_pos * b->lev_mask_bytes + (size_t)b->n_win * 4 + cov_bytes + clon_bytes + rare_bytes + s.sat_rows.size() * sizeof(isx_sat));
    }
    {
        const int lrc = finish_pass_link(b, sfin);
        if (lrc != ISX_OK) return lrc;
        if (!(p->prm.enable_linkage && b->link_chain == 3)) HIP_TRY(isx_read_sync(sfin));
    }
    t_fin = now_ms();
    if (dense && p->prm.rarefied_coverage > 0) {
        const size_t n_rare = b->n_rare;
        isx_rare *rr = reinterpret_cast<isx_rare *>(s.h_small + s.o_rare);
        s.rare_big.clear();
        s.rare_dense = false;
        if (n_rare > p->cap_rare || n_rare * 8 > (size_t)b->n_pos) {
            if (!p->pp.want_counts) {
                if (s.clonr_big.size() < (size_t)b->n_pos) s.clonr_big.resize((size_t)b->n_pos);
                if (p->bounce[0]) { const int rc = bounce_d2h(p, s.clonr_big.data(), b->d_clon_r, (size_t)b->n_pos * 4, sfin); if (rc != ISX_OK) return rc; }
                else HIP_TRY(hipMemcpy(s.clonr_big.data(), b->d_clon_r, (size_t)b->n_pos * 4, hipMemcpyDeviceToHost));
            } else if (redo && s.out_pinned)
                HIP_TRY(hipMemcpy(s.h_out + s.o_clonr, b->d_clon_r, (size_t)b->n_pos * 4, hipMemcpyDeviceToHost));
            s.rare_dense = true;
        } else {
            if (n_rare > p->rare_prefix || redo) {
                if (n_rare > p->rare_prefix) { s.rare_big.resize(n_rare); rr = s.rare_big.data(); }
                { const int prc = pull(rr, b->d_rare, n_rare * sizeof(isx_rare)); if (prc != ISX_OK) return prc; }
            }
            if (!b->ordered) std::sort(rr, rr + n_rare, [](const isx_rare &x, const isx_rare &y) { return x.gpos < y.gpos; });
        }
    }
    t_rare = now_ms();
    const size_t n_snv = (size_t)b->sizes.n_snv;
    isx_snv *rows = reinterpret_cast<isx_snv *>(s.h_small + s.o_snv);
    if (n_snv > p->snv_prefix || redo) {
        if (n_snv > p->snv_prefix) { s.snv_big.resize(n_snv); rows = s.snv_big.data(); }
        { const int prc = pull(rows, b->d_snv, n_snv * sizeof(isx_snv)); if (prc != ISX_OK) return prc; }
    }
    if (!b->ordered) std::sort(rows, rows + n_snv, [](const isx_snv &x, const isx_snv &y) { return x.gpos != y.gpos ? x.gpos < y.gpos : x.mm < y.mm; });
    if (p->prm.enable_linkage) {
        s.ld_rows.resize((size_t)b->sizes.n_ld);
        if (!s.ld_rows.empty() && b->ld_host && s.ld_rows.size() <= b->n_ld_host) memcpy(s.ld_rows.data(), b->ld_host, s.ld_rows.size() * sizeof(isx_ld));
        else if (!s.ld_rows.empty()) { const int rc = pull(s.ld_rows.data(), b->L.ld.p, s.ld_rows.size() * sizeof(isx_ld)); if (rc != ISX_OK) return rc; }
    }
    s.rows_checksum = bytes_checksum(s.ld_rows.data(), p->prm.enable_linkage ? s.ld_rows.size() * sizeof(isx_ld) : 0, bytes_checksum(rows, n_snv * sizeof(isx_snv), 0));
    if (pipe_timing)
        fprintf(stderr, "[isx_pipe finisher] wait %.2f ms, finish (sizes, linkage) %.2f ms [device: sites %.2f allele %.2f group %.2f incr %.2f ld %.2f; %lld ao, %lld incr, %lld ld], clonTR list (%u) %.2f ms, snv rows (%zu) %.2f ms\n",
                s.finish_wait_ms, t_fin - t_c0, b->tim.sites_ms, b->tim.allele_ms, b->tim.group_ms, b->tim.incr_ms, b->tim.ld_ms,
                (long long)b->sizes.n_allele_obs, (long long)b->sizes.n_increments, (long long)b->sizes.n_ld, b->n_rare, t_rare - t_fin, n_snv, now_ms() - t_rare);
    return ISX_OK;
}

static void finisher_main(isx_pipe *p, hipStream_t sfin)
{
    (void)hipSetDevice(p->ctx->device);
    for (;;) {
        int64_t ticket;
        {
            std::unique_lock<std::mutex> lk(p->mu);
            p->cv_work.wait(lk, [&] { return p->stop || !p->work.empty(); });
            if (p->work.empty()) return;
            ticket = p->work.front();
            p->work.pop_front();
        }
        Slot &s = p->slots[(size_t)(ticket % (int64_t)p->slots.size())];
        const int rc = finish_slot(p, s, sfin);
        std::string err = rc == ISX_OK ? std::string() : std::string(isx_last_error());
        BamBatch *dead = nullptr;
        {
            std::lock_guard<std::mutex> lk(p->mu);
            s.rc = rc; s.err.swap(err);
            dead = s.dead_batch; s.dead_batch = nullptr;
            s.state = 2;
        }
        p->cv_done.notify_all();
        if (dead) bam_batch_retire(dead);
    }
}

static int submit_segs_common(isx_pipe *p, int64_t n_pos, const uint8_t *ref, int32_t n_splits, const int64_t *split_bounds,
                              isxenc::SegJob &J, int64_t *ticket, const isx_ref_planes *rp = nullptr);

static void stager_main(isx_pipe *p)
{
    for (;;) {
        isx_pipe::StageJob job;
        {
            std::unique_lock<std::mutex> lk(p->mu);
// ... 93 lines not shown
    const double t_c0 = now_ms();
    p->pool.reset(new isxenc::HostPool(nt, gpu_numa_node(c->device), pp->pin_threads != 0));
    const double t_c1 = now_ms();
    int rc = ISX_OK;
    hipError_t e;
    if ((e = isx_side_stream_create(c, &p->s_h2d)) != hipSuccess ||
        (e = isx_side_stream_create(c, &p->s_fin)) != hipSuccess ||
        (e = isx_side_stream_create(c, &p->s_fin2)) != hipSuccess ||
        (e = isx_side_stream_create(c, &p->s_d2h)) != hipSuccess) {
        isx_set_error(std::string("isx_pipe_create: ") + hipGetErrorString(e));
        pipe_free(p);
        return ISX_ERR_HIP;
    }
    p->slots.resize((size_t)pp->depth);
    {
        const char *e2 = getenv("ISX_PIPE_H2D_STREAMS");
        if (e2 && atoi(e2) >= 2 && pp->depth >= 2 && isx_side_stream_create(c, &p->s_h2d2) != hipSuccess) { p->s_h2d2 = nullptr; (void)hipGetLastError(); }
    }
    for (int i = 0; i < pp->depth && rc == ISX_OK; i++) {
        rc = slot_batch_create(p, p->slots[(size_t)i], i);
        if ((i & 1) && p->s_h2d2) p->slots[(size_t)i].h2d = p->s_h2d2;
    }
    if (rc != ISX_OK) { pipe_free(p); return rc; }
    if (!p->slots[0].out_pinned) {
        p->bounce_bytes = (size_t)16 << 20;
        for (int i = 0; i < 2 && rc == ISX_OK; i++) {
            if (isx_pin_malloc(reinterpret_cast<void **>(&p->bounce[i]), p->bounce_bytes) != hipSuccess ||
                hipEventCreateWithFlags(&p->bounce_ev[i], hipEventDisableTiming) != hipSuccess) rc = ISX_ERR_HIP;
        }
        if (rc != ISX_OK) { isx_set_error("isx_pipe_create: bounce buffers"); pipe_free(p); return rc; }
        p->fin_pool.reset(new isxenc::HostPool(std::max(1, std::min(nt, 6)), -1, false));
    }
    p->finisher = std::thread(finisher_main, p, p->s_fin);
    if (pp->depth >= 2) p->finisher2 = std::thread(finisher_main, p, p->s_fin2);
    {
        int want = pp->depth >= 4 ? 4 : 2;
        if (const char *e = getenv("ISX_PIPE_FINISHERS")) want = std::max(1, atoi(e));
        want = std::min(want, pp->depth);
        for (int i = 2; i < want; i++) {
            hipStream_t st = nullptr;
            if (isx_side_stream_create(c, &st) != hipSuccess) break;
            p->extra_fin.push_back(st);
            p->more_finishers.emplace_back(finisher_main, p, st);
        }
    }
    if (pipe_timing)
        fprintf(stderr, "[isx_pipe_create] thread pool %.1f ms, %d slot(s) %.1f ms\n", t_c1 - t_c0, pp->depth, now_ms() - t_c1);
    if (pp->stage_async && p->segs) p->stager = std::thread(stager_main, p);
    *out = p;
    return ISX_OK;
}

void isx_pipe_destroy(isx_pipe *p) { pipe_free(p); }

static int enqueue_pass_impl(isx_pipe *p, Slot &s, int64_t n_pos, int64_t *ticket);

static int enqueue_pass(isx_pipe *p, Slot &s, int64_t n_pos, int64_t *ticket)
{
    const int rc = enqueue_pass_impl(p, s, n_pos, ticket);
    if (rc != ISX_OK) {
        const std::string why(isx_last_error());
        (void)isx_wait_stream(H2D(p, s));
        (void)isx_wait_stream(p->ctx->pstream[s.b->ps]);
        (void)isx_wait_stream(p->s_d2h);
        isx_set_error(why);
    }
    return rc;
}

static int enqueue_pass_impl(isx_pipe *p, Slot &s, int64_t n_pos, int64_t *ticket)
{
    isx_ctx *c = p->ctx;
    isx_batch *b = s.b;
    const bool dense = b->M == 1, linkage = p->prm.enable_linkage != 0;
    hipStream_t ps = c->pstream[b->ps];
    int rc = ISX_OK;
    std::unique_lock<std::mutex> launch_lk(p->launch_mu);
    HIP_TRY(hipStreamWaitEvent(ps, s.ev_h2d1, 0));
    if (dense && p->prm.rarefied_coverage > 0 && b->rare_dense)
        HIP_TRY(hipMemsetD32Async(reinterpret_cast<hipDeviceptr_t>(b->d_clon_r), 0x7FC00000, (size_t)n_pos, ps));
    if (linkage && p->rb == 4)
        launch_extract_gpos(nullptr, b->d_rec32, b->d_gbase, nullptr, b->d_gpos16, b->d_gbase, ISX_GROUP, b->n_rec, ps);
    if ((rc = launch_pass(b)) != ISX_OK) return rc;
    {
        PileupArgs pa{};
        pa.cursors = b->d_cursors; pa.host_state = b->d_host_state;
        launch_publish_state(pa, b->epoch, ps);
        b->publish_enqueued = true;
        if (c->unpublished[b->ps] == b) c->unpublished[b->ps] = nullptr;
    }
    HIP_TRY(hipEventRecord(s.ev_pass, ps));

    HIP_TRY(hipStreamWaitEvent(p->s_d2h, s.ev_pass, 0));
    HIP_TRY(hipEventRecord(s.ev_d2h0, p->s_d2h));
    const size_t snv_rows = std::min(p->snv_prefix, b->cap_snv);
    HIP_TRY(isx_copy_rows_to_host(s.h_small + s.o_snv, b->d_snv, b->d_cursors + CUR_SNV, b->base[CUR_SNV], (uint32_t)sizeof(isx_snv), snv_rows, p->s_d2h));
    s.d2h_bytes = 0;
    if (dense) {
        if (p->prm.rarefied_coverage > 0) {
            const size_t n = std::min(p->rare_prefix, std::min(p->cap_rare, (size_t)n_pos));
            HIP_TRY(isx_copy_rows_to_host(s.h_small + s.o_rare, b->d_rare, b->d_cursors + CUR_RARE, b->base[CUR_RARE], (uint32_t)sizeof(isx_rare), n, p->s_d2h));
        }
        if (!b->sparse_out) s.d2h_bytes += (int64_t)n_pos * 6;
    }
    if (dense && s.out_pinned && !b->sparse_out) {
        HIP_TRY(isx_copy_to_host(s.h_out + s.o_cov16, b->d_cov16, (size_t)n_pos * 2, p->s_d2h));
        HIP_TRY(isx_copy_to_host(s.h_out + s.o_clon, b->d_clon, (size_t)n_pos * 4, p->s_d2h));
        if (p->pp.want_counts) {
            HIP_TRY(isx_copy_to_host(s.h_out + s.o_counts, b->d_counts, (size_t)n_pos * 16, p->s_d2h));
            s.d2h_bytes += (int64_t)n_pos * 16;
            if (p->prm.rarefied_coverage > 0) {
                HIP_TRY(isx_copy_to_host(s.h_out + s.o_clonr, b->d_clon_r, (size_t)n_pos * 4, p->s_d2h));
                s.d2h_bytes += (int64_t)n_pos * 4;
            }
        }
    }
    HIP_TRY(hipEventRecord(s.ev_d2h1, p->s_d2h));
    launch_lk.unlock();
    {
        std::lock_guard<std::mutex> lk(p->mu);
        s.ticket = p->next_ticket++;
        if (p->next_promise < p->next_ticket) p->next_promise = p->next_ticket;
        s.state = 1; s.rc = ISX_OK;
        *ticket = s.ticket;
        p->work.push_back(s.ticket);
    }
    p->cv_work.notify_one();
    return ISX_OK;
}


static int check_capacity(const isx_pipe *p, const char *who, int64_t n_pos, int64_t n_items, int64_t max_items, int32_t n_splits)
{
    if (n_pos > p->pp.max_pos || n_items > max_items || n_splits > p->pp.max_splits) {
        isx_set_error(std::string(who) + ": batch larger than the pipe was created for");
        return ISX_ERR_CAPACITY;
    }
    return ISX_OK;
}

static int slot_acquire(isx_pipe *p, const char *who, Slot **out)
{
    Slot &s = p->slots[(size_t)(p->next_ticket % (int64_t)p->slots.size())];
    {
        std::lock_guard<std::mutex> lk(p->mu);
        if (s.state != 0) { isx_set_error(std::string(who) + ": every slot is in use (collect + release the oldest batch first)"); return ISX_ERR_STATE; }
    }
    HIP_TRY(hipSetDevice(p->ctx->device));
    *out = &s;
    return ISX_OK;
}

static int queue_for_stager(isx_pipe *p, isx_pipe::StageJob &&job, const char *who, int64_t *ticket)
{
    const int rc = check_capacity(p, who, job.n_pos, job.planes ? job.reads.n_seg : job.segs.n_seg, p->pp.max_segs, (int32_t)job.bounds.size() - 1);
    if (rc != ISX_OK) return rc;
    {
        std::lock_guard<std::mutex> lk(p->mu);
        const int64_t t = p->next_promise, n = (int64_t)p->slots.size();
        const Slot &s = p->slots[(size_t)(t % n)];
        if (t - n >= p->next_ticket || s.state != 0) { isx_set_error(std::string(who) + ": every slot is in use (collect + release the oldest batch first)"); return ISX_ERR_STATE; }
        job.ticket = t;
        p->next_promise = t + 1;
        *ticket = t;
        p->stage_q.push_back(std::move(job));
    }
    p->cv_stage.notify_one();
    return ISX_OK;
}

struct RingFeed { hipError_t err = hipSuccess; size_t bytes = 0; };

static int ring_feed_install(isx_pipe *p, Slot &s, RingFeed &r, int64_t &ring_groups, std::function<void(int)> &wave_begin,
                             std::function<void(int, int64_t, int64_t)> &wave_flush)
{
    if (p->ring_half <= 0) return ISX_OK;
    HIP_TRY(hipEventRecord(s.ev_h2d0, H2D(p, s)));
    const size_t half_bytes = (size_t)p->ring_half * (size_t)p->rb, grp_bytes = (size_t)p->G * (size_t)p->rb;
    uint8_t *d_rec = s.d_in + s.off_rec;
    ring_groups = p->ring_half / (int64_t)p->G;
    wave_begin = [&s, &r](int h) {
        if (s.ring_busy[h]) { const hipError_t e = isx_wait_event(s.ev_ring[h]); if (e != hipSuccess && r.err == hipSuccess) r.err = e; s.ring_busy[h] = false; }
    };
    wave_flush = [p, &s, &r, half_bytes, grp_bytes, d_rec](int h, int64_t g0, int64_t g1) {
        const size_t n = (size_t)(g1 - g0) * grp_bytes;
        if (g0 == 0) r.bytes = 0;
        hipError_t e = hipMemcpyAsync(d_rec + (size_t)g0 * grp_bytes, s.h_in + s.off_rec + (size_t)h * half_bytes, n, hipMemcpyHostToDevice, H2D(p, s));
// ... 860 lines not shown
```

Before: 170.2.

## Enqueue linkage chain on device before host readback and fuse hand-back copies

The linkage bucket-chain stage is now launched on the D2H stream right after the pileup pass. It reads site and allele-observation counts from the device cursors instead of waiting for host-side sizes, and a head prefix of LD rows is copied into pinned memory. The separate publish-state kernel and the row copies for SNV, rare and LD are merged into one hand-back kernel. This is meant to remove a host round trip and several small launches between the pass and linkage, letting linkage overlap with finalisation. In exchange it adds device-side capacity checks with a fallback path, and more state is carried across the enqueue and finish steps.

```diff
diff --git a/instrain_amd/csrc/isx_api.hip b/instrain_amd/csrc/isx_api.hip
--- a/instrain_amd/csrc/isx_api.hip
+++ b/instrain_amd/csrc/isx_api.hip
@@ -275,6 +275,55 @@
     const int blocks = (int)std::min<size_t>(64, (n16 + 1023) / 1024);
     hipLaunchKernelGGL(k_copy_counted, dim3(std::max(blocks, 1)), dim3(256), 0, stream, static_cast<uint4 *>(hdst), static_cast<const uint4 *>(dsrc),
                        d_cursor, base, row_bytes, (uint64_t)cap_rows);
+    return hipGetLastError();
+}
+
+namespace {
+struct RowJobs {
+    uint4 *dst[ISX_ROW_JOBS]; const uint4 *src[ISX_ROW_JOBS]; const uint32_t *count[ISX_ROW_JOBS];
+    uint32_t base[ISX_ROW_JOBS], row_bytes[ISX_ROW_JOBS], head_rows[ISX_ROW_JOBS], first[ISX_ROW_JOBS + 1];
+    uint64_t cap_rows[ISX_ROW_JOBS];
+    int n;
+    const uint32_t *cursors; uint32_t *host_state; uint32_t epoch;
+};
+__global__ void __launch_bounds__(256) k_hand_back(const RowJobs J)
+{
+    if (blockIdx.x == J.first[J.n]) {
+        const int i = threadIdx.x;
+        if (i < CUR_N + 4) J.host_state[i] = __hip_atomic_load(&J.cursors[i], __ATOMIC_RELAXED, __HIP_MEMORY_SCOPE_AGENT);
+        __threadfence_system();
+        __syncthreads();
+        if (i == 0) __hip_atomic_store(&J.host_state[CUR_N + 4], J.epoch, __ATOMIC_RELEASE, __HIP_MEMORY_SCOPE_SYSTEM);
+        return;
+    }
+    int j = 0;
+    while (j + 1 < J.n && blockIdx.x >= J.first[j + 1]) j++;
+    const uint32_t nb = J.first[j + 1] - J.first[j], lb = blockIdx.x - J.first[j];
+    const uint64_t rows = (uint64_t)J.head_rows[j] + min((uint64_t)(*J.count[j] - J.base[j]), J.cap_rows[j]);
+    const uint64_t n16 = (rows * J.row_bytes[j] + 15) / 16;
+    uint4 *__restrict__ dst = J.dst[j];
+    const uint4 *__restrict__ src = J.src[j];
+    for (uint64_t i = (uint64_t)lb * 256u + threadIdx.x; i < n16; i += (uint64_t)nb * 256u) dst[i] = src[i];
+}
+}
+
+hipError_t isx_hand_back(const isx_row_job *jobs, int n, const uint32_t *d_cursors, uint32_t *d_host_state, uint32_t epoch, hipStream_t stream)
+{
+    RowJobs J{};
+    uint32_t blocks = 0;
+    for (int i = 0; i < n; i++) {
+        if (!jobs[i].cap_rows && !jobs[i].head_rows) continue;
+        if (J.n == ISX_ROW_JOBS || ((reinterpret_cast<uintptr_t>(jobs[i].dst) | reinterpret_cast<uintptr_t>(jobs[i].src)) & 15) != 0) return hipErrorInvalidValue;
+        const size_t n16 = ((jobs[i].cap_rows + jobs[i].head_rows) * jobs[i].row_bytes + 15) / 16;
+        J.dst[J.n] = static_cast<uint4 *>(jobs[i].dst); J.src[J.n] = static_cast<const uint4 *>(jobs[i].src); J.count[J.n] = jobs[i].count;
+        J.base[J.n] = jobs[i].base; J.row_bytes[J.n] = jobs[i].row_bytes; J.head_rows[J.n] = jobs[i].head_rows; J.cap_rows[J.n] = jobs[i].cap_rows;
+        J.first[J.n] = blocks;
+        blocks += (uint32_t)std::max<size_t>(1, std::min<size_t>(64, (n16 + 1023) / 1024));
+        J.n++;
+    }
+    J.first[J.n] = blocks;
+    J.cursors = d_cursors; J.host_state = d_host_state; J.epoch = epoch;
+    hipLaunchKernelGGL(k_hand_back, dim3(blocks + 1), dim3(256), 0, stream, J);
     return hipGetLastError();
 }
 
@@ -1412,20 +1461,47 @@
     return ISX_OK;
 }
 
-int finish_pass_link(isx_batch *b, hipStream_t link_stream)
+static void link_in_of_batch(isx_batch *b, hipStream_t s, LinkageIn &in)
+{
+    isx_ctx *c = b->ctx;
+    in.stream = s; in.ev = &b->ev[2]; in.ev_mfma = &b->ev[8];
+    in.mode = b->prm.linkage_mode == 2 ? 2 : 1;
+    in.philox = Philox{(uint32_t)b->prm.seed, (uint32_t)(b->prm.seed >> 32)};
+    in.n_pairs = b->n_pairs; in.ao = b->d_ao;
+    in.sites = b->d_sites; in.sites_ordered = b->ordered;
+    in.slev = b->d_slev; in.snv = b->d_snv;
+    in.split_bounds = b->d_bounds; in.n_splits = b->n_splits; in.M = b->M; in.min_snp = b->prm.min_snp;
+    in.d_cursors = b->d_cursors; in.cap_sites = b->cap_sites; in.cap_ao = b->cap_ao;
+    in.grid = 8 * (c->pass_cus < 256 ? 256 - c->pass_cus : 256);
+}
+
+int enqueue_pass_link(isx_batch *b, hipStream_t s, isx_row_job *job)
+{
+    b->L.enqueued = false;
+    if (!b->prm.enable_linkage) return ISX_OK;
+    LinkageIn in{};
+    link_in_of_batch(b, s, in);
+    in.base_sites = b->base[CUR_SITES]; in.base_ao = b->base[CUR_AO];
+    const isx_ld *blk = nullptr;
+    const uint32_t *n_rows = nullptr;
+    size_t prefix = 0;
+    const int rc = link_chain_enqueue(in, b->L, &blk, &n_rows, &prefix);
+    if (rc != ISX_OK || !b->L.enqueued) return rc;
+    *job = isx_row_job{nullptr, blk, n_rows, 0u, (uint32_t)sizeof(isx_ld), (uint32_t)LD_HEAD, prefix};
+    return ISX_OK;
+}
+
+int finish_pass_link(isx_batch *b, hipStream_t link_stream, const void *prefetched)
 {
     isx_ctx *c = b->ctx;
     hipStream_t s = link_stream ? link_stream : c->stream;
     if (b->prm.enable_linkage) {
         LinkageIn in{};
-        in.stream = s; in.ev = &b->ev[2]; in.ev_mfma = &b->ev[8];
-        in.mode = b->prm.linkage_mode == 2 ? 2 : 1;
-        in.philox = Philox{(uint32_t)b->prm.seed, (uint32_t)(b->prm.seed >> 32)};
-        in.n_pairs = b->n_pairs; in.ao = b->d_ao; in.n_ao = b->n_ao_pass;
-        in.sites = b->d_sites; in.n_sites = (uint32_t)b->sizes.n_sites; in.sites_ordered = b->ordered;
-        in.slev = b->d_slev; in.snv = b->d_snv;
+        link_in_of_batch(b, s, in);
+        in.n_ao = b->n_ao_pass; in.n_sites = (uint32_t)b->sizes.n_sites;
+        in.base_sites = b->base[CUR_SITES] - in.n_sites; in.base_ao = b->base[CUR_AO] - in.n_ao;
+        in.prefetched = static_cast<const isx_ld *>(prefetched);
         if (b->M > 1 && b->d_win_site_cnt && !b->sites_loose) { in.win_site_base = b->d_win_site_base; in.win_site_cnt = b->d_win_site_cnt; in.n_win = b->n_win; }
-        in.split_bounds = b->d_bounds; in.n_splits = b->n_splits; in.M = b->M; in.min_snp = b->prm.min_snp;
         LinkageOut lo;
         int rc = run_linkage(in, b->L, lo);
         if (rc != ISX_OK) return rc;
diff --git a/instrain_amd/csrc/isx_batch.h b/instrain_amd/csrc/isx_batch.h
--- a/instrain_amd/csrc/isx_batch.h
+++ b/instrain_amd/csrc/isx_batch.h
@@ -146,6 +146,7 @@
 int launch_pass(isx_batch *b);
 int finish_pass(isx_batch *b, uint32_t *cap_flags, hipStream_t link_stream = nullptr);
 int finish_pass_sizes(isx_batch *b, uint32_t *cap_flags, hipStream_t link_stream = nullptr);
-int finish_pass_link(isx_batch *b, hipStream_t link_stream = nullptr);
+int finish_pass_link(isx_batch *b, hipStream_t link_stream = nullptr, const void *prefetched = nullptr);
+int enqueue_pass_link(isx_batch *b, hipStream_t s, isx_row_job *job);
 int batch_grow_tables(isx_batch *b, uint32_t cap_flags);
 }
diff --git a/instrain_amd/csrc/isx_internal.h b/instrain_amd/csrc/isx_internal.h
--- a/instrain_amd/csrc/isx_internal.h
+++ b/instrain_amd/csrc/isx_internal.h
@@ -34,6 +34,9 @@
 hipError_t isx_copy_to_host_route(void *hdst_pinned, const void *dsrc, size_t bytes, hipStream_t stream, bool by_kernel);
 hipError_t isx_copy_rows_to_host(void *hdst_pinned, const void *dsrc, const uint32_t *d_cursor, uint32_t base, uint32_t row_bytes,
                                  size_t cap_rows, hipStream_t stream);
+#define ISX_ROW_JOBS 4
+struct isx_row_job { void *dst; const void *src; const uint32_t *count; uint32_t base, row_bytes, head_rows; size_t cap_rows; };
+hipError_t isx_hand_back(const isx_row_job *jobs, int n, const uint32_t *d_cursors, uint32_t *d_host_state, uint32_t epoch, hipStream_t stream);
 bool isx_host_is_registered(const void *ptr, size_t bytes);
 hipError_t isx_read_back(void *host_dst, const void *dsrc, size_t bytes, hipStream_t stream);
 hipError_t isx_read_sync(hipStream_t stream);
diff --git a/instrain_amd/csrc/isx_linkage.h b/instrain_amd/csrc/isx_linkage.h
--- a/instrain_amd/csrc/isx_linkage.h
+++ b/instrain_amd/csrc/isx_linkage.h
@@ -36,6 +36,16 @@
     DevBuf<uint64_t> edge_list;
     uint32_t chain_epoch = 0;
     std::vector<isx_ld> h_ld;
+    struct Chain {
+        uint32_t lim_sites = 0, lim_ao = 0;
+        size_t cap_keys = 0, cap_ld = 0;
+        size_t test_keys = 0, test_ld = 0;
+        uint32_t max_u = 0;
+        int logH = 12;
+        bool direct = false;
+        const isx_site *sites_sorted = nullptr;
+    } chain;
+    bool enqueued = false;
     DevBuf<uint64_t> key64, key64b;
     DevBuf<uint32_t> head, row_id, first_row, first_site, split_slot, tile_cnt, tile_off, vals, vals2;
     DevBuf<DenseSplit> dsplits;
@@ -53,6 +63,11 @@
     uint32_t n_ao;
     const isx_site *sites;
     uint32_t n_sites;
+    const uint32_t *d_cursors = nullptr;
+    uint32_t base_sites = 0, base_ao = 0;
+    size_t cap_sites = 0, cap_ao = 0;
+    int grid = 0;
+    const isx_ld *prefetched = nullptr;
     bool sites_ordered = false;
     const uint32_t *win_site_base = nullptr, *win_site_cnt = nullptr;
     int n_win = 0;
@@ -75,3 +90,5 @@
 };
 
 int run_linkage(const LinkageIn &in, LinkageBuffers &B, LinkageOut &out);
+
+int link_chain_enqueue(const LinkageIn &in, LinkageBuffers &B, const isx_ld **ld_block, const uint32_t **n_rows, size_t *prefix_rows);
diff --git a/instrain_amd/csrc/isx_linkage.hip b/instrain_amd/csrc/isx_linkage.hip
--- a/instrain_amd/csrc/isx_linkage.hip
+++ b/instrain_amd/csrc/isx_linkage.hip
@@ -248,55 +248,156 @@
 constexpr uint64_t LK_EMPTY = ~0ull;
 constexpr uint32_t LK_STAGE = 256;
 constexpr uint32_t LK_ROUND = 16;
-enum { LS_NINC = 0, LS_NU = 1, LS_NEDGES = 2, LS_NLD = 3, LS_FLAGS = 4, LS_NLIST1 = 5 , LS_NLIST2 = 6 , LS_WORDS = 16 };
-constexpr uint32_t LKF_KEYS = 1u, LKF_BUCKET = 2u, LKF_LD = 4u;
-
-__global__ void __launch_bounds__(256) k_link_prep(const isx_site *sites, uint32_t n, const int64_t *bounds, int n_splits,
-                                                   uint32_t *site_gpos, uint32_t *site_split, uint32_t *site_cnt, uint32_t *site_rows, uint32_t *state)
-{
-    const uint32_t i = blockIdx.x * blockDim.x + threadIdx.x;
-    if (i < LS_WORDS) state[i] = 0;
-    if (i >= n) return;
-    const uint32_t g = sites[i].gpos;
-    int lo = 0, hi = n_splits;
-    while (hi - lo > 1) {
-        const int mid = (lo + hi) >> 1;
-        if (bounds[mid] <= (int64_t)g) lo = mid; else hi = mid;
-    }
-    site_gpos[i] = g;
-    site_split[i] = (uint32_t)lo;
-    site_cnt[i] = 0;
-    site_rows[i] = 0;
-}
-
-__global__ void __launch_bounds__(256) k_ao_chain(isx_ao *ao, uint32_t n, const uint32_t *site_gpos, uint32_t n_sites,
-                                                  unsigned long long *head, int hshift, uint32_t direct, uint32_t epoch, uint32_t *next)
-{
-    const uint32_t i = blockIdx.x * blockDim.x + threadIdx.x;
-    if (i >= n) return;
-    const uint32_t g = ao[i].site;
-    uint32_t lo = 0, hi = n_sites;
-    while (lo < hi) {
-        const uint32_t mid = (lo + hi) >> 1;
-        if (site_gpos[mid] < g) lo = mid + 1; else hi = mid;
-    }
-    ao[i].site = lo;
-    const uint32_t pr = ao[i].pair;
-    const uint32_t h = pr < direct ? pr : (pr * 0x9E3779B1u) >> hshift;
-    const unsigned long long old = atomicExch(&head[h], ((unsigned long long)epoch << 32) | i);
-    next[i] = (uint32_t)(old >> 32) == epoch ? (uint32_t)old : LK_NIL;
+enum { LS_NINC = 0, LS_NU = 1, LS_NEDGES = 2, LS_NLD = 3, LS_FLAGS = 4, LS_NLIST1 = 5 , LS_NLIST2 = 6 ,
+       LS_TICKET1 = 7, LS_TICKET2 = 8 ,
+       LS_NSITES = 9, LS_NAO = 10 , LS_WORDS = 16 };
+constexpr uint32_t LKF_KEYS = 1u, LKF_BUCKET = 2u, LKF_LD = 4u, LKF_SIZE = 8u ;
+
+struct LkCounts {
+    const uint32_t *cur;
+    uint32_t base_sites, base_ao;
+    uint32_t cap_sites, cap_ao;
+    uint32_t lim_sites, lim_ao;
+};
+
+__global__ void __launch_bounds__(256) k_link_prep(const LkCounts c, const isx_site *sites, const int64_t *bounds, int n_splits,
+                                                   uint32_t *site_gpos, uint32_t *site_split, uint32_t *site_cnt, uint32_t *site_rows, uint32_t *state,
+                                                   isx_ao *ao, unsigned long long *head, int hshift, uint32_t direct, uint32_t epoch, uint32_t *next)
+{
+    const bool pass_ok = (c.cur[CUR_N] & ~ISX_FLAG_SITES_LOOSE) == 0;
+    uint32_t n_sites = pass_ok ? min(c.cur[CUR_SITES] - c.base_sites, c.cap_sites) : 0u;
+    uint32_t n_ao = pass_ok ? min(c.cur[CUR_AO] - c.base_ao, c.cap_ao) : 0u;
+    const bool fits = n_sites <= c.lim_sites && n_ao <= c.lim_ao;
+    if (!fits) { n_sites = 0; n_ao = 0; }
+    const uint32_t gi = blockIdx.x * blockDim.x + threadIdx.x, stride = gridDim.x * blockDim.x;
+    if (gi < LS_WORDS) state[gi] = gi == LS_NSITES ? n_sites : (gi == LS_NAO ? n_ao : (gi == LS_FLAGS && !fits ? LKF_SIZE : 0u));
+    for (uint64_t i = gi; i < n_sites; i += stride) {
+        const uint32_t g = sites[i].gpos;
+        int lo = 0, hi = n_splits;
+        while (hi - lo > 1) {
+            const int mid = (lo + hi) >> 1;
+            if (bounds[mid] <= (int64_t)g) lo = mid; else hi = mid;
+        }
+        site_gpos[i] = g;
+        site_split[i] = (uint32_t)lo;
+        site_cnt[i] = 0;
+        site_rows[i] = 0;
+    }
+    for (uint64_t i = gi; i < n_ao; i += stride) {
+        const uint32_t g = ao[i].site;
+        uint32_t lo = 0, hi = n_sites;
+        while (lo < hi) {
+            const uint32_t mid = (lo + hi) >> 1;
+            if (sites[mid].gpos < g) lo = mid + 1; else hi = mid;
+        }
+        ao[i].site = lo;
+        const uint32_t pr = ao[i].pair;
+        const uint32_t h = pr < direct ? pr : (pr * 0x9E3779B1u) >> hshift;
+        const unsigned long long old = atomicExch(&head[h], ((unsigned long long)epoch << 32) | (uint32_t)i);
+        next[i] = (uint32_t)(old >> 32) == epoch ? (uint32_t)old : LK_NIL;
+    }
+}
+
+template <int NT>
+__device__ __forceinline__ void lk_scan_block(const uint32_t *in, uint32_t *out, uint32_t n, uint32_t *total, uint32_t *zero,
+                                              uint32_t *list, uint32_t *n_list)
+{
+    constexpr int SUB = 1024 / NT, NW = NT / 64;
+    __shared__ uint32_t wsum[16], wnz[16];
+    __shared__ uint32_t carry_s, carry_nz;
+    __shared__ unsigned long long total_s;
+    const uint32_t t = threadIdx.x, l = t & 63, w = t >> 6;
+    if (t == 0) { carry_s = 0; carry_nz = 0; total_s = 0; }
+    __syncthreads();
+    auto load4 = [&](uint32_t i0) -> uint4 {
+        if (i0 + 4 <= n) return *reinterpret_cast<const uint4 *>(in + i0);
+        uint4 x;
+        x.x = i0 < n ? in[i0] : 0u; x.y = i0 + 1 < n ? in[i0 + 1] : 0u; x.z = i0 + 2 < n ? in[i0 + 2] : 0u; x.w = 0u;
+        return x;
+    };
+    uint4 nxt = load4(4 * t);
+    for (uint32_t base = 0; base < n; base += 4096) {
+        uint32_t inc[SUB], inz[SUB];
+        uint4 x[SUB];
+#pragma unroll
+        for (int q = 0; q < SUB; q++) x[q] = (SUB == 1) ? nxt : load4(base + 4 * ((uint32_t)q * NT + t));
+        if (SUB == 1 && base + 4096 < n) nxt = load4(base + 4 * t + 4096);
+#pragma unroll
+        for (int q = 0; q < SUB; q++) {
+            inc[q] = x[q].x + x[q].y + x[q].z + x[q].w;
+            inz[q] = (x[q].x != 0) + (x[q].y != 0) + (x[q].z != 0) + (x[q].w != 0);
+#pragma unroll
+            for (int d = 1; d < 64; d <<= 1) {
+                const uint32_t o = __shfl_up(inc[q], d), oz = __shfl_up(inz[q], d);
+                if ((int)l >= d) { inc[q] += o; inz[q] += oz; }
+            }
+            if (l == 63) { wsum[q * NW + w] = inc[q]; wnz[q * NW + w] = inz[q]; }
+        }
+        __syncthreads();
+        uint32_t run = 0, rnz = 0;
+#pragma unroll
+        for (int q = 0; q < SUB; q++) {
+            const uint32_t i0 = base + 4 * ((uint32_t)q * NT + t);
+            const uint4 y = (SUB == 1) ? x[q] : load4(i0);
+            const uint32_t v[4] = {y.x, y.y, y.z, y.w};
+            const uint32_t mine = v[0] + v[1] + v[2] + v[3], mine_nz = (v[0] != 0) + (v[1] != 0) + (v[2] != 0) + (v[3] != 0);
+            uint32_t before = carry_s, before_nz = carry_nz;
+            for (uint32_t r = 0; r < (uint32_t)q * NW + w; r++) { before += wsum[r]; before_nz += wnz[r]; }
+            run = before + inc[q] - mine; rnz = before_nz + inz[q] - mine_nz;
+            uint4 o;
+            o.x = run; o.y = run + v[0]; o.z = o.y + v[1]; o.w = o.z + v[2];
+            run = o.w + v[3];
+            if (i0 + 4 <= n) {
+                *reinterpret_cast<uint4 *>(out + i0) = o;
+                if (zero) *reinterpret_cast<uint4 *>(zero + i0) = make_uint4(0, 0, 0, 0);
+            } else {
+                if (i0 < n) { out[i0] = o.x; if (zero) zero[i0] = 0; }
+                if (i0 + 1 < n) { out[i0 + 1] = o.y; if (zero) zero[i0 + 1] = 0; }
+                if (i0 + 2 < n) { out[i0 + 2] = o.z; if (zero) zero[i0 + 2] = 0; }
+            }
+#pragma unroll
+            for (int e = 0; e < 4; e++) if (v[e] != 0) list[rnz++] = i0 + e;
+        }
+        __syncthreads();
+        if (t == NT - 1) { total_s += (unsigned long long)(run - carry_s); carry_s = run; carry_nz = rnz; }
+        __syncthreads();
+    }
+    if (t == 0) { const uint32_t tot = total_s > 0xFFFFFFFEull ? 0xFFFFFFFFu : (uint32_t)total_s; out[n] = tot; *total = tot; *n_list = carry_nz; }
+}
+
+__global__ void __launch_bounds__(1024) k_scan_u32(const uint32_t *in, uint32_t *out, uint32_t n, uint32_t *total, uint32_t *zero,
+                                                   uint32_t *list, uint32_t *n_list)
+{
+    lk_scan_block<1024>(in, out, n, total, zero, list, n_list);
+}
+
+__device__ __forceinline__ bool lk_last_block(uint32_t *ticket)
+{
+    __shared__ uint32_t last_s;
+    __threadfence();
+    __syncthreads();
+    if (threadIdx.x == 0) {
+        last_s = atomicAdd(ticket, 1u) == gridDim.x - 1 ? 1u : 0u;
+        if (last_s) atomicExch(ticket, 0u);
+    }
+    __syncthreads();
+    const bool last = last_s != 0;
+    if (last) __threadfence();
+    return last;
 }
 
 template <bool EMIT>
-__global__ void __launch_bounds__(256) k_pair_walk(const isx_ao *ao, uint32_t n, const uint32_t *next, const uint32_t *site_split,
-                                                   uint32_t *site_cnt, const uint32_t *site_off, uint64_t *keys, uint64_t cap_keys,
-                                                   uint32_t *state)
-{
-    const uint32_t i = blockIdx.x * blockDim.x + threadIdx.x, l = threadIdx.x & 63;
+__global__ void __launch_bounds__(256) k_pair_walk(const isx_ao *ao, const uint32_t *next, const uint32_t *site_split,
+                                                   uint32_t *site_cnt, uint32_t *site_off, uint64_t *keys, uint64_t cap_keys,
+                                                   uint32_t *state, uint32_t *site_cur, uint32_t *site_list)
+{
+    const uint32_t n = state[LS_NAO], l = threadIdx.x & 63;
     if (EMIT && (uint64_t)state[LS_NINC] > cap_keys) {
-        if (i == 0) atomicOr(&state[LS_FLAGS], LKF_KEYS);
+        if (blockIdx.x == 0 && threadIdx.x == 0) atomicOr(&state[LS_FLAGS], LKF_KEYS);
         return;
     }
+    for (uint64_t i0 = (uint64_t)blockIdx.x * blockDim.x; i0 < n; i0 += (uint64_t)gridDim.x * blockDim.x) {
+    const uint32_t i = (uint32_t)i0 + threadIdx.x;
     isx_ao a{};
     uint32_t sa = 0, j = LK_NIL;
     if (i < n) { a = ao[i]; sa = site_split[a.site]; j = next[i]; }
@@ -332,60 +433,11 @@
         }
         if (EMIT && hit) keys[site_off[s1] + slot] = key;
     }
-}
-
-__global__ void __launch_bounds__(1024) k_scan_u32(const uint32_t *in, uint32_t *out, uint32_t n, uint32_t *total, uint32_t *zero,
-                                                   uint32_t *list, uint32_t *n_list)
-{
-    __shared__ uint32_t wsum[16], wnz[16];
-    __shared__ uint32_t carry_s, carry_nz;
-    __shared__ unsigned long long total_s;
-    const uint32_t t = threadIdx.x, l = t & 63, w = t >> 6;
-    if (t == 0) { carry_s = 0; carry_nz = 0; total_s = 0; }
-    __syncthreads();
-    auto load4 = [&](uint32_t i0) -> uint4 {
-        if (i0 + 4 <= n) return *reinterpret_cast<const uint4 *>(in + i0);
-        uint4 x;
-        x.x = i0 < n ? in[i0] : 0u; x.y = i0 + 1 < n ? in[i0 + 1] : 0u; x.z = i0 + 2 < n ? in[i0 + 2] : 0u; x.w = 0u;
-        return x;
-    };
-    uint4 nxt = load4(4 * t);
-    for (uint32_t base = 0; base < n; base += 4096) {
-        const uint32_t i0 = base + 4 * t;
-        const uint4 x = nxt;
-        if (base + 4096 < n) nxt = load4(i0 + 4096);
-        const uint32_t v[4] = {x.x, x.y, x.z, x.w};
-        const uint32_t mine = v[0] + v[1] + v[2] + v[3];
-        const uint32_t mine_nz = (v[0] != 0) + (v[1] != 0) + (v[2] != 0) + (v[3] != 0);
-        uint32_t inc = mine, inz = mine_nz;
-#pragma unroll
-        for (int d = 1; d < 64; d <<= 1) {
-            const uint32_t o = __shfl_up(inc, d), oz = __shfl_up(inz, d);
-            if ((int)l >= d) { inc += o; inz += oz; }
-        }
-        if (l == 63) { wsum[w] = inc; wnz[w] = inz; }
-        __syncthreads();
-        uint32_t before = carry_s, before_nz = carry_nz;
-        for (uint32_t q = 0; q < w; q++) { before += wsum[q]; before_nz += wnz[q]; }
-        uint32_t run = before + inc - mine, rnz = before_nz + inz - mine_nz;
-        uint4 o;
-        o.x = run; o.y = run + v[0]; o.z = o.y + v[1]; o.w = o.z + v[2];
-        run = o.w + v[3];
-        if (i0 + 4 <= n) {
-            *reinterpret_cast<uint4 *>(out + i0) = o;
-            if (zero) *reinterpret_cast<uint4 *>(zero + i0) = make_uint4(0, 0, 0, 0);
-        } else {
-            if (i0 < n) { out[i0] = o.x; if (zero) zero[i0] = 0; }
-            if (i0 + 1 < n) { out[i0 + 1] = o.y; if (zero) zero[i0 + 1] = 0; }
-            if (i0 + 2 < n) { out[i0 + 2] = o.z; if (zero) zero[i0 + 2] = 0; }
-        }
-#pragma unroll
-        for (int q = 0; q < 4; q++) if (v[q] != 0) list[rnz++] = i0 + q;
-        __syncthreads();
-        if (t == 1023) { total_s += (unsigned long long)(run - carry_s); carry_s = run; carry_nz = rnz; }
-        __syncthreads();
-    }
-    if (t == 0) { const uint32_t tot = total_s > 0xFFFFFFFEull ? 0xFFFFFFFFu : (uint32_t)total_s; out[n] = tot; *total = tot; *n_list = carry_nz; }
+    }
+    if (!EMIT) {
+        if (lk_last_block(&state[LS_TICKET1]))
+            lk_scan_block<256>(site_cnt, site_off, state[LS_NSITES], state + LS_NINC, site_cur, site_list, state + LS_NLIST1);
+    }
 }
 
 __device__ __forceinline__ uint32_t lk_hash(uint64_t k) { return (uint32_t)((k * 0x9E3779B97F4A7C15ull) >> 40); }
@@ -598,8 +650,8 @@
 
 template <bool EMIT>
 __global__ void __launch_bounds__(256) k_edge_rows(const uint64_t *keys, const uint32_t *ucnt, uint32_t *rows_per, const uint32_t *site_off,
-                                                   const uint32_t *site_nu, uint32_t *site_rows, const uint32_t *site_row_off, const uint2 *edge_list,
-                                                   SiteView v, int min_snp, isx_ld *out, uint64_t cap_ld, uint32_t *state, Philox ph)
+                                                   const uint32_t *site_nu, uint32_t *site_rows, uint32_t *site_row_off, const uint2 *edge_list,
+                                                   SiteView v, int min_snp, isx_ld *out, uint64_t cap_ld, uint32_t *state, Philox ph, uint32_t *site_list)
 {
     if (state[LS_FLAGS] & (LKF_KEYS | LKF_BUCKET)) return;
     if (EMIT && (uint64_t)state[LS_NLD] > cap_ld) { if (blockIdx.x == 0 && threadIdx.x == 0) atomicOr(&state[LS_FLAGS], LKF_LD); return; }
@@ -617,6 +669,10 @@
             for (uint32_t q = 0; q < u; q++) before += rows_per[off + q];
             (void)ld_edge_rows<true>(keys + off, ucnt + off, u, nu, s1, s2, v, min_snp, out + before, ph);
         }
+    }
+    if (!EMIT) {
+        if (lk_last_block(&state[LS_TICKET2]))
+            lk_scan_block<256>(site_rows, site_row_off, state[LS_NSITES], state + LS_NLD, (uint32_t *)nullptr, site_list, state + LS_NLIST2);
     }
 }
 
@@ -902,16 +958,27 @@
     return ISX_OK;
 }
 
-int bucket_chain(const LinkageIn &in, LinkageBuffers &B, LinkageOut &out, const isx_site *sites_sorted, bool *fell_back)
+int chain_prepare(const LinkageIn &in, LinkageBuffers &B, const isx_site *sites_sorted, bool known)
 {
     hipStream_t s = in.stream;
     int rc;
-    *fell_back = false;
-    const uint32_t n_ao = in.n_ao, n_sites = in.n_sites;
-    const bool direct = in.n_pairs && in.n_pairs <= 8ull * n_ao + (1ull << 20) && in.n_pairs <= (1ull << 31);
-    int logH = 12;
-    while (logH < 31 && (1ull << logH) < (direct ? in.n_pairs : 2ull * n_ao)) logH++;
-    const size_t H = (size_t)1 << logH;
+    LinkageBuffers::Chain &C = B.chain;
+    const size_t first = (size_t)1 << 20;
+    const size_t need_sites = std::max<size_t>(C.lim_sites, known ? in.n_sites : std::min<size_t>(in.cap_sites ? in.cap_sites : first, first));
+    const size_t need_ao = std::max<size_t>(C.lim_ao, known ? in.n_ao : std::min<size_t>(in.cap_ao ? in.cap_ao : first, first));
+    if ((rc = ensure(B.site_gpos, need_sites + 1)) || (rc = ensure(B.site_split, need_sites + 1)) || (rc = ensure(B.next, need_ao)) ||
+        (rc = ensure(B.site_cnt, need_sites + 1)) || (rc = ensure(B.site_off, need_sites + 1)) || (rc = ensure(B.site_cur, need_sites + 1)) ||
+        (rc = ensure(B.site_nu, need_sites + 1)) || (rc = ensure(B.site_rows, need_sites + 1)) || (rc = ensure(B.site_row_off, need_sites + 1)) ||
+        (rc = ensure(B.site_list1, need_sites + 1)) || (rc = ensure(B.site_list2, need_sites + 1))) return rc;
+    size_t hold = B.site_gpos.cap;
+    for (size_t c : {B.site_split.cap, B.site_cnt.cap, B.site_off.cap, B.site_cur.cap, B.site_nu.cap, B.site_rows.cap, B.site_row_off.cap,
+                     B.site_list1.cap, B.site_list2.cap}) hold = std::min(hold, c);
+    C.lim_sites = (uint32_t)std::min<size_t>(hold - 1, (1u << 26) - 1);
+    C.lim_ao = (uint32_t)std::min<size_t>(B.next.cap, 0xFFFFFFFEu);
+    C.direct = in.n_pairs && in.n_pairs <= 8ull * C.lim_ao + (1ull << 20) && in.n_pairs <= (1ull << 31);
+    C.logH = 12;
+    while (C.logH < 31 && (1ull << C.logH) < (C.direct ? in.n_pairs : 2ull * C.lim_ao)) C.logH++;
+    const size_t H = (size_t)1 << C.logH;
     if (B.chain_head.cap < H || !B.chain_head.p) {
         if ((rc = ensure(B.chain_head, H))) return rc;
         HIP_TRY(hipMemsetAsync(B.chain_head.p, 0, B.chain_head.cap * sizeof(uint64_t), s));
@@ -921,85 +988,126 @@
         HIP_TRY(hipMemsetAsync(B.chain_head.p, 0, B.chain_head.cap * sizeof(uint64_t), s));
         B.chain_epoch = 1;
     }
-    size_t cap_keys = std::max<size_t>(B.keys.cap, std::max<size_t>((size_t)n_ao * 2, 65536));
-    size_t cap_ld = std::max<size_t>(B.ld_block.cap > LD_HEAD ? B.ld_block.cap - LD_HEAD : 0, 4096);
+    C.cap_keys = std::max<size_t>(B.keys.cap, std::max<size_t>((known ? (size_t)in.n_ao : (size_t)C.lim_ao) * 2, 65536));
+    C.cap_ld = std::max<size_t>(B.ld_block.cap > LD_HEAD ? B.ld_block.cap - LD_HEAD : 0, 4096);
     static_assert(sizeof(isx_ld) * LD_HEAD >= LS_WORDS * sizeof(uint32_t), "the state words fit the head of ld_block");
-    uint32_t max_u = LK_MAXU;
-    if (const char *e = getenv("ISX_LINK_MAXU")) max_u = (uint32_t)std::min<long>(std::max<long>(atol(e), 1), LK_MAXU);
-    size_t test_keys = 0, test_ld = 0;
-    if (const char *e = getenv("ISX_LINK_TEST_CAPS")) { unsigned long a = 0, b = 0; if (sscanf(e, "%lu,%lu", &a, &b) == 2) { test_keys = a; test_ld = b; } }
-    auto size_tables = [&]() -> int {
-        int r;
-        if ((r = ensure(B.keys, cap_keys)) || (r = ensure(B.ucnt, cap_keys)) || (r = ensure(B.rows_per, cap_keys)) || (r = ensure(B.edge_list, cap_keys))) return r;
-        cap_keys = std::min(std::min(B.keys.cap, B.ucnt.cap), std::min(B.rows_per.cap, B.edge_list.cap));
-        return ISX_OK;
-    };
-    auto size_ld = [&]() -> int {
-        const int r = ensure_ld(B, cap_ld);
-        if (r) return r;
-        cap_ld = B.ld.cap;
-        return ISX_OK;
-    };
-    if ((rc = ensure(B.next, n_ao)) || (rc = ensure(B.site_cnt, (size_t)n_sites + 1)) || (rc = ensure(B.site_off, (size_t)n_sites + 1)) ||
-        (rc = ensure(B.site_cur, (size_t)n_sites + 1)) || (rc = ensure(B.site_nu, n_sites)) || (rc = ensure(B.site_rows, (size_t)n_sites + 1)) ||
-        (rc = ensure(B.site_row_off, (size_t)n_sites + 1)) || (rc = ensure(B.site_list1, n_sites)) || (rc = ensure(B.site_list2, n_sites)) || (rc = size_tables()) || (rc = size_ld())) return rc;
+    C.max_u = LK_MAXU;
+    if (const char *e = getenv("ISX_LINK_MAXU")) C.max_u = (uint32_t)std::min<long>(std::max<long>(atol(e), 1), LK_MAXU);
+    C.test_keys = C.test_ld = 0;
+    if (const char *e = getenv("ISX_LINK_TEST_CAPS")) { unsigned long a = 0, b = 0; if (sscanf(e, "%lu,%lu", &a, &b) == 2) { C.test_keys = a; C.test_ld = b; } }
+    C.sites_sorted = sites_sorted;
+    return ISX_OK;
+}
+
+int chain_size_tables(LinkageBuffers &B)
+{
+    int r;
+    LinkageBuffers::Chain &C = B.chain;
+    if ((r = ensure(B.keys, C.cap_keys)) || (r = ensure(B.ucnt, C.cap_keys)) || (r = ensure(B.rows_per, C.cap_keys)) || (r = ensure(B.edge_list, C.cap_keys))) return r;
+    C.cap_keys = std::min(std::min(B.keys.cap, B.ucnt.cap), std::min(B.rows_per.cap, B.edge_list.cap));
+    return ISX_OK;
+}
+
+int chain_size_ld(LinkageBuffers &B)
+{
+    const int r = ensure_ld(B, B.chain.cap_ld);
+    if (r) return r;
+    B.chain.cap_ld = B.ld.cap;
+    return ISX_OK;
+}
+
+int chain_launch(const LinkageIn &in, LinkageBuffers &B, int stage, bool first)
+{
+    hipStream_t s = in.stream;
+    const LinkageBuffers::Chain &C = B.chain;
     uint32_t *state = reinterpret_cast<uint32_t *>(B.ld_block.p);
-    const dim3 blk(256), g_sites((n_sites + 255) / 256), g_ao((n_ao + 255) / 256);
-    SiteView v{sites_sorted, in.slev, in.snv, in.M == 1 ? 1 : 0};
-    hipLaunchKernelGGL(k_link_prep, g_sites, blk, 0, s, sites_sorted, n_sites, in.split_bounds, in.n_splits, B.site_gpos.p, B.site_split.p,
-                       B.site_cnt.p, B.site_rows.p, state);
-    EV(1);
-    hipLaunchKernelGGL(k_ao_chain, g_ao, blk, 0, s, in.ao, n_ao, B.site_gpos.p, n_sites, reinterpret_cast<unsigned long long *>(B.chain_head.p),
-                       32 - logH, direct ? (uint32_t)H : 0u, B.chain_epoch, B.next.p);
-    EV(2);
-    hipLaunchKernelGGL((k_pair_walk<false>), g_ao, blk, 0, s, in.ao, n_ao, B.next.p, B.site_split.p, B.site_cnt.p, nullptr, nullptr, (uint64_t)0, state);
-    hipLaunchKernelGGL(k_scan_u32, dim3(1), dim3(1024), 0, s, B.site_cnt.p, B.site_off.p, n_sites, state + LS_NINC, B.site_cur.p, B.site_list1.p, state + LS_NLIST1);
-    const dim3 g_waves(std::min<uint32_t>((n_sites + LK_ROUND - 1) / LK_ROUND, 4096)), g_edges(std::min<uint32_t>((uint32_t)std::min<size_t>((cap_keys + 255) / 256, 0x7FFFFFFF), 2048));
+    const uint32_t g = (uint32_t)std::min(std::max(in.grid > 0 ? in.grid : 512, 64), 4096);
+    const dim3 blk(256), grid(g), g_waves(std::min<uint32_t>(4 * g, 4096));
+    SiteView v{C.sites_sorted, in.slev, in.snv, in.M == 1 ? 1 : 0};
+    if (stage == 0) {
+        LkCounts c{in.d_cursors, in.base_sites, in.base_ao, (uint32_t)std::min<size_t>(in.cap_sites, 0xFFFFFFFFu), (uint32_t)std::min<size_t>(in.cap_ao, 0xFFFFFFFFu),
+                   C.lim_sites, C.lim_ao};
+        hipLaunchKernelGGL(k_link_prep, grid, blk, 0, s, c, C.sites_sorted, in.split_bounds, in.n_splits, B.site_gpos.p, B.site_split.p,
+                           B.site_cnt.p, B.site_rows.p, state, in.ao, reinterpret_cast<unsigned long long *>(B.chain_head.p),
+                           32 - C.logH, C.direct ? (uint32_t)((size_t)1 << C.logH) : 0u, B.chain_epoch, B.next.p);
+        EV(1);
+        EV(2);
+        hipLaunchKernelGGL((k_pair_walk<false>), grid, blk, 0, s, in.ao, B.next.p, B.site_split.p, B.site_cnt.p, B.site_off.p, (uint64_t *)nullptr, (uint64_t)0,
+                           state, B.site_cur.p, B.site_list1.p);
+    }
+    if (stage <= 1) {
+        hipLaunchKernelGGL((k_pair_walk<true>), grid, blk, 0, s, in.ao, B.next.p, B.site_split.p, B.site_cur.p, B.site_off.p, B.keys.p,
+                           (uint64_t)(first && C.test_keys ? std::min(C.test_keys, C.cap_keys) : C.cap_keys), state, (uint32_t *)nullptr, (uint32_t *)nullptr);
+        EV(3);
+        hipLaunchKernelGGL(k_site_edges, g_waves, dim3(64), 0, s, B.keys.p, B.ucnt.p, B.rows_per.p, B.site_off.p, B.site_nu.p,
+                           reinterpret_cast<uint2 *>(B.edge_list.p), state, C.max_u, B.site_list1.p);
+        hipLaunchKernelGGL((k_edge_rows<false>), grid, blk, 0, s, B.keys.p, B.ucnt.p, B.rows_per.p, B.site_off.p, B.site_nu.p, B.site_rows.p,
+                           B.site_row_off.p, reinterpret_cast<const uint2 *>(B.edge_list.p), v, in.min_snp, (isx_ld *)nullptr, (uint64_t)0, state, in.philox, B.site_list2.p);
+        EV(4);
+    }
+    hipLaunchKernelGGL((k_edge_rows<true>), grid, blk, 0, s, B.keys.p, B.ucnt.p, B.rows_per.p, B.site_off.p, B.site_nu.p, B.site_rows.p,
+                       B.site_row_off.p, reinterpret_cast<const uint2 *>(B.edge_list.p), v, in.min_snp, B.ld.p,
+                       (uint64_t)(first && C.test_ld ? std::min(C.test_ld, C.cap_ld) : C.cap_ld), state, in.philox, (uint32_t *)nullptr);
+    EV(5);
+    HIP_TRY(hipGetLastError());
+    return ISX_OK;
+}
+
+int bucket_chain(const LinkageIn &in, LinkageBuffers &B, LinkageOut &out, const isx_site *sites_sorted, bool enqueued, bool *fell_back)
+{
+    hipStream_t s = in.stream;
+    int rc;
+    *fell_back = false;
+    LinkageBuffers::Chain &C = B.chain;
+    if (!enqueued) {
+        if ((rc = chain_prepare(in, B, sites_sorted, true)) || (rc = chain_size_tables(B)) || (rc = chain_size_ld(B)) || (rc = chain_launch(in, B, 0, true))) return rc;
+    }
     uint32_t h[LS_WORDS] = {0};
-    for (int stage = 0, attempt = 0;; attempt++) {
-        if (attempt == 4) { isx_set_error("linkage tables still too small after three growth steps"); return ISX_ERR_CAPACITY; }
-        if (stage == 0) {
-            hipLaunchKernelGGL((k_pair_walk<true>), g_ao, blk, 0, s, in.ao, n_ao, B.next.p, B.site_split.p, B.site_cur.p, B.site_off.p, B.keys.p,
-                               (uint64_t)(attempt == 0 && test_keys ? std::min(test_keys, cap_keys) : cap_keys), state);
-            EV(3);
-            hipLaunchKernelGGL(k_site_edges, g_waves, dim3(64), 0, s, B.keys.p, B.ucnt.p, B.rows_per.p, B.site_off.p, B.site_nu.p,
-                               reinterpret_cast<uint2 *>(B.edge_list.p), state, max_u, B.site_list1.p);
-            hipLaunchKernelGGL((k_edge_rows<false>), g_edges, blk, 0, s, B.keys.p, B.ucnt.p, B.rows_per.p, B.site_off.p, B.site_nu.p, B.site_rows.p,
-                               (const uint32_t *)nullptr, reinterpret_cast<const uint2 *>(B.edge_list.p), v, in.min_snp, (isx_ld *)nullptr, (uint64_t)0, state, in.philox);
-            hipLaunchKernelGGL(k_scan_u32, dim3(1), dim3(1024), 0, s, B.site_rows.p, B.site_row_off.p, n_sites, state + LS_NLD, (uint32_t *)nullptr, B.site_list2.p, state + LS_NLIST2);
-            EV(4);
-        }
-        hipLaunchKernelGGL((k_edge_rows<true>), g_edges, blk, 0, s, B.keys.p, B.ucnt.p, B.rows_per.p, B.site_off.p, B.site_nu.p, B.site_rows.p,
-                           B.site_row_off.p, reinterpret_cast<const uint2 *>(B.edge_list.p), v, in.min_snp, B.ld.p,
-                           (uint64_t)(attempt == 0 && test_ld ? std::min(test_ld, cap_ld) : cap_ld), state, in.philox);
-        HIP_TRY(hipGetLastError());
-        const size_t n_pre = std::min<size_t>(cap_ld, LD_PREFIX_ROWS);
+    for (int attempt = 0;; attempt++) {
+        if (attempt == 5) { isx_set_error("linkage tables still too small after four growth steps"); return ISX_ERR_CAPACITY; }
+        const size_t n_pre = std::min<size_t>(C.cap_ld, LD_PREFIX_ROWS);
         B.h_ld.resize(LD_HEAD + n_pre);
-        HIP_TRY(isx_read_back(B.h_ld.data(), B.ld_block.p, (LD_HEAD + n_pre) * sizeof(isx_ld), s));
-        EV(5);
-        HIP_TRY(isx_read_sync(s));
-        memcpy(h, B.h_ld.data(), sizeof(h));
+        if (enqueued && attempt == 0 && in.prefetched) {
+            memcpy(h, in.prefetched, sizeof(h));
+            const size_t rows = (h[LS_FLAGS] & (LKF_SIZE | LKF_KEYS | LKF_BUCKET | LKF_LD)) ? 0 : std::min<size_t>(h[LS_NLD], n_pre);
+            memcpy(B.h_ld.data(), in.prefetched, (LD_HEAD + rows) * sizeof(isx_ld));
+        } else {
+            HIP_TRY(isx_read_back(B.h_ld.data(), B.ld_block.p, (LD_HEAD + n_pre) * sizeof(isx_ld), s));
+            HIP_TRY(isx_read_sync(s));
+            memcpy(h, B.h_ld.data(), sizeof(h));
+        }
+        if (h[LS_FLAGS] & LKF_SIZE) {
+            if (!enqueued || attempt != 0) { isx_set_error("internal: the linkage chain's arrays do not hold the batch they were sized for"); return ISX_ERR_STATE; }
+            if ((rc = chain_prepare(in, B, sites_sorted, true)) || (rc = chain_size_tables(B)) || (rc = chain_size_ld(B)) || (rc = chain_launch(in, B, 0, false))) return rc;
+            continue;
+        }
+        if (h[LS_NSITES] != in.n_sites || h[LS_NAO] != in.n_ao) {
+            isx_set_error("internal: the linkage chain ran with other sizes than the pass reported (" + std::to_string(h[LS_NSITES]) + " / " + std::to_string(h[LS_NAO]) +
+                          " against " + std::to_string(in.n_sites) + " sites / " + std::to_string(in.n_ao) + " observations)");
+            return ISX_ERR_STATE;
+        }
+        uint32_t *state = reinterpret_cast<uint32_t *>(B.ld_block.p);
         if (h[LS_FLAGS] & LKF_KEYS) {
             if (h[LS_NINC] == 0xFFFFFFFFu) { isx_set_error("more than 2^32 pair increments in one batch"); return ISX_ERR_CAPACITY; }
-            cap_keys = (size_t)h[LS_NINC] + h[LS_NINC] / 4 + 4096;
+            C.cap_keys = (size_t)h[LS_NINC] + h[LS_NINC] / 4 + 4096;
             B.keys.cap = B.ucnt.cap = B.rows_per.cap = B.edge_list.cap = 0;
-            if ((rc = size_tables())) return rc;
+            if ((rc = chain_size_tables(B))) return rc;
             HIP_TRY(hipMemsetAsync(state + LS_NU, 0, (LS_FLAGS + 1 - LS_NU) * sizeof(uint32_t), s));
-            HIP_TRY(hipMemsetAsync(B.site_cur.p, 0, ((size_t)n_sites + 1) * sizeof(uint32_t), s));
-            stage = 0;
+            HIP_TRY(hipMemsetAsync(B.site_cur.p, 0, ((size_t)in.n_sites + 1) * sizeof(uint32_t), s));
+            if ((rc = chain_launch(in, B, 1, false))) return rc;
             continue;
         }
         if (h[LS_FLAGS] & LKF_BUCKET) { *fell_back = true; return ISX_OK; }
         if (h[LS_FLAGS] & LKF_LD) {
             if (h[LS_NLD] == 0xFFFFFFFFu) { isx_set_error("more than 2^32 LD rows in one batch"); return ISX_ERR_CAPACITY; }
-            cap_ld = (size_t)h[LS_NLD] + h[LS_NLD] / 4 + 4096;
+            C.cap_ld = (size_t)h[LS_NLD] + h[LS_NLD] / 4 + 4096;
             B.ld_block.cap = 0;
-            if ((rc = size_ld())) return rc;
+            if ((rc = chain_size_ld(B))) return rc;
             state = reinterpret_cast<uint32_t *>(B.ld_block.p);
             h[LS_FLAGS] &= ~LKF_LD;
             HIP_TRY(hipMemcpyAsync(state, h, sizeof(h), hipMemcpyHostToDevice, s));
             HIP_TRY(isx_wait_stream(s));
-            stage = 1;
+            if ((rc = chain_launch(in, B, 2, false))) return rc;
             continue;
         }
         break;
@@ -1122,30 +1230,58 @@
 
 }
 
+static bool chain_sorted_by_env()
+{
+    const char *chain_env = getenv("ISX_LINK_CHAIN");
+    return chain_env && !strcmp(chain_env, "sorted");
+}
+
+int link_chain_enqueue(const LinkageIn &in, LinkageBuffers &B, const isx_ld **ld_block, const uint32_t **n_rows, size_t *prefix_rows)
+{
+    hipStream_t s = in.stream;
+    int rc;
+    B.enqueued = false;
+    if (in.mode == 2 || !in.sites_ordered || in.M > 256 || !in.d_cursors || chain_sorted_by_env()) return ISX_OK;
+    EV(0);
+    HIP_TRY(hipEventRecord(in.ev_mfma[0], s));
+    HIP_TRY(hipEventRecord(in.ev_mfma[1], s));
+    if ((rc = chain_prepare(in, B, in.sites, false)) || (rc = chain_size_tables(B)) || (rc = chain_size_ld(B)) || (rc = chain_launch(in, B, 0, true))) return rc;
+    B.enqueued = true;
+    *ld_block = B.ld_block.p;
+    *n_rows = reinterpret_cast<const uint32_t *>(B.ld_block.p) + LS_NLD;
+    *prefix_rows = std::min<size_t>(B.chain.cap_ld, LD_PREFIX_ROWS);
+    return ISX_OK;
+}
+
 int run_linkage(const LinkageIn &in, LinkageBuffers &B, LinkageOut &out)
 {
     hipStream_t s = in.stream;
     out = LinkageOut();
     const uint32_t n_sites = in.n_sites;
     int rc;
+    const bool enqueued = B.enqueued;
+    B.enqueued = false;
     const bool lt = getenv("ISX_LINK_TIMING") != nullptr;
     const auto lt0 = std::chrono::steady_clock::now();
     auto tick = [&](const char *what) {
         if (lt) fprintf(stderr, "[run_linkage] %-22s +%.2f ms\n", what, std::chrono::duration<double, std::milli>(std::chrono::steady_clock::now() - lt0).count());
     };
-    EV(0);
-    HIP_TRY(hipEventRecord(in.ev_mfma[0], s));
-    HIP_TRY(hipEventRecord(in.ev_mfma[1], s));
-    if (n_sites == 0) { EV(1); EV(2); EV(3); EV(4); EV(5); return ISX_OK; }
+    if (!enqueued) {
+        EV(0);
+        HIP_TRY(hipEventRecord(in.ev_mfma[0], s));
+        HIP_TRY(hipEventRecord(in.ev_mfma[1], s));
+        if (n_sites == 0) { EV(1); EV(2); EV(3); EV(4); EV(5); return ISX_OK; }
+    }
     if (n_sites >= (1u << 26)) { isx_set_error("more than 2^26 SNP sites in one batch: split the batch"); return ISX_ERR_ARG; }
     if (in.M > 256) { isx_set_error("linkage supports at most 256 mm bins"); return ISX_ERR_ARG; }
     if (in.mode == 2 && in.M != 1) { isx_set_error("the dense MFMA linkage path needs n_mm_bins == 1"); return ISX_ERR_ARG; }
 
+    const isx_site *sites_sorted = in.sites;
+    if (!enqueued) {
     if ((rc = ensure(B.site_keys, n_sites)) || (rc = ensure(B.site_keys2, n_sites)) ||
         (rc = ensure(B.sites_sorted, n_sites)) || (rc = ensure(B.site_gpos, n_sites)) ||
         (rc = ensure(B.site_split, n_sites))) return rc;
     tick("site buffers");
-    const isx_site *sites_sorted = in.sites;
     const char *site_env = getenv("ISX_LINK_SITE_SORT");
     if (!in.sites_ordered && in.win_site_cnt && in.n_win > 0 && !(site_env && !strcmp(site_env, "rocprim"))) {
         if ((rc = ensure(B.win_off, (size_t)in.n_win + 1)) || (rc = ensure(B.win_list, (size_t)in.n_win)) || (rc = ensure(B.n_runs, 2))) return rc;
@@ -1159,14 +1295,14 @@
                                      B.sites_sorted.p, n_sites, 0, 32, s));
         sites_sorted = B.sites_sorted.p;
     }
+    } else sites_sorted = B.chain.sites_sorted;
     const uint32_t n_ao = in.n_ao;
     out.n_ao = n_ao;
-    const char *chain_env = getenv("ISX_LINK_CHAIN");
-    const bool bucket = in.mode != 2 && n_ao != 0 && !(chain_env && !strcmp(chain_env, "sorted"));
+    const bool bucket = enqueued || (in.mode != 2 && n_ao != 0 && !chain_sorted_by_env());
     bool ranked = false;
     if (bucket) {
         bool fell_back = false;
-        if ((rc = bucket_chain(in, B, out, sites_sorted, &fell_back)) != ISX_OK) return rc;
+        if ((rc = bucket_chain(in, B, out, sites_sorted, enqueued, &fell_back)) != ISX_OK) return rc;
         tick("bucket chain");
         if (!fell_back) { out.chain = 3; return ISX_OK; }
         ranked = true;
diff --git a/instrain_amd/csrc/isx_pipe.hip b/instrain_amd/csrc/isx_pipe.hip
--- a/instrain_amd/csrc/isx_pipe.hip
+++ b/instrain_amd/csrc/isx_pipe.hip
@@ -61,7 +61,7 @@
     uint8_t *h_small = nullptr;
     size_t small_bytes = 0;
     bool out_pinned = true;
-    size_t out_bytes = 0, o_counts = 0, o_clon = 0, o_clonr = 0, o_snv = 0, o_cov16 = 0, o_rare = 0;
+    size_t out_bytes = 0, o_counts = 0, o_clon = 0, o_clonr = 0, o_snv = 0, o_cov16 = 0, o_rare = 0, o_link = 0;
     bool rare_dense = false;
     bool cov8 = false, clon_sparse = false;
     bool cov4 = false;
@@ -464,6 +464,7 @@
     o = 0;
     s.o_snv = o; o = up(o + p->snv_prefix * sizeof(isx_snv));
     s.o_rare = o; if (dense && prm->rarefied_coverage > 0) o = up(o + p->rare_prefix * sizeof(isx_rare));
+    s.o_link = o; if (prm->enable_linkage) o = up(o + (LD_HEAD + LD_PREFIX_ROWS) * sizeof(isx_ld));
     s.small_bytes = o;
     HIP_TRY(isx_pin_malloc(reinterpret_cast<void **>(&s.h_small), std::max<size_t>(s.small_bytes, 1)));
     o = 0;
@@ -558,6 +559,7 @@
         }
         redo = true;
     }
+    if (redo) b->L.enqueued = false;
     s.d2h_bytes += (int64_t)(std::min((size_t)b->sizes.n_snv, p->snv_prefix) * sizeof(isx_snv));
     if (dense && p->prm.rarefied_coverage > 0) s.d2h_bytes += (int64_t)(std::min((size_t)b->n_rare, p->rare_prefix) * sizeof(isx_rare));
     auto pull = [&](void *hdst, const void *dsrc, size_t bytes) -> int {
@@ -646,7 +648,11 @@
         if (!s.sat_rows.empty()) HIP_TRY(isx_read_back(s.sat_rows.data(), b->d_sat, s.sat_rows.size() * sizeof(isx_sat), sfin));
         s.d2h_bytes += (int64_t)((size_t)b->n_pos * b->lev_mask_bytes + (size_t)b->n_win * 4 + cov_bytes + clon_bytes + rare_bytes + s.sat_rows.size() * sizeof(isx_sat));
     }
-    {
+    if (p->prm.enable_linkage && b->L.enqueued) {
+        HIP_TRY(isx_read_sync(sfin));
+        const int lrc = finish_pass_link(b, sfin, s.h_small + s.o_link);
+        if (lrc != ISX_OK) return lrc;
+    } else {
         const int lrc = finish_pass_link(b, sfin);
         if (lrc != ISX_OK) return lrc;
         if (!(p->prm.enable_linkage && b->link_chain == 3)) HIP_TRY(isx_read_sync(sfin));
@@ -906,27 +912,30 @@
     if (linkage && p->rb == 4)
         launch_extract_gpos(nullptr, b->d_rec32, b->d_gbase, nullptr, b->d_gpos16, b->d_gbase, ISX_GROUP, b->n_rec, ps);
     if ((rc = launch_pass(b)) != ISX_OK) return rc;
-    {
-        PileupArgs pa{};
-        pa.cursors = b->d_cursors; pa.host_state = b->d_host_state;
-        launch_publish_state(pa, b->epoch, ps);
-        b->publish_enqueued = true;
-        if (c->unpublished[b->ps] == b) c->unpublished[b->ps] = nullptr;
-    }
+    b->publish_enqueued = true;
+    if (c->unpublished[b->ps] == b) c->unpublished[b->ps] = nullptr;
     HIP_TRY(hipEventRecord(s.ev_pass, ps));
 
     HIP_TRY(hipStreamWaitEvent(p->s_d2h, s.ev_pass, 0));
     HIP_TRY(hipEventRecord(s.ev_d2h0, p->s_d2h));
+    isx_row_job jobs[3];
+    int n_jobs = 0;
+    if (linkage) {
+        isx_row_job lj{};
+        if ((rc = enqueue_pass_link(b, p->s_d2h, &lj)) != ISX_OK) return rc;
+        if (b->L.enqueued) { lj.dst = s.h_small + s.o_link; jobs[n_jobs++] = lj; }
+    }
     const size_t snv_rows = std::min(p->snv_prefix, b->cap_snv);
-    HIP_TRY(isx_copy_rows_to_host(s.h_small + s.o_snv, b->d_snv, b->d_cursors + CUR_SNV, b->base[CUR_SNV], (uint32_t)sizeof(isx_snv), snv_rows, p->s_d2h));
+    jobs[n_jobs++] = isx_row_job{s.h_small + s.o_snv, b->d_snv, b->d_cursors + CUR_SNV, b->base[CUR_SNV], (uint32_t)sizeof(isx_snv), 0u, snv_rows};
     s.d2h_bytes = 0;
     if (dense) {
         if (p->prm.rarefied_coverage > 0) {
             const size_t n = std::min(p->rare_prefix, std::min(p->cap_rare, (size_t)n_pos));
-            HIP_TRY(isx_copy_rows_to_host(s.h_small + s.o_rare, b->d_rare, b->d_cursors + CUR_RARE, b->base[CUR_RARE], (uint32_t)sizeof(isx_rare), n, p->s_d2h));
+            jobs[n_jobs++] = isx_row_job{s.h_small + s.o_rare, b->d_rare, b->d_cursors + CUR_RARE, b->base[CUR_RARE], (uint32_t)sizeof(isx_rare), 0u, n};
         }
         if (!b->sparse_out) s.d2h_bytes += (int64_t)n_pos * 6;
     }
+    HIP_TRY(isx_hand_back(jobs, n_jobs, b->d_cursors, b->d_host_state, b->epoch, p->s_d2h));
     if (dense && s.out_pinned && !b->sparse_out) {
         HIP_TRY(isx_copy_to_host(s.h_out + s.o_cov16, b->d_cov16, (size_t)n_pos * 2, p->s_d2h));
         HIP_TRY(isx_copy_to_host(s.h_out + s.o_clon, b->d_clon, (size_t)n_pos * 4, p->s_d2h));
```

New measurement: 169.0. No clear change (-0.7%).
